# nitishsaDire/objectDetection_ssd

Hardware: AMD Instinct MI355X
Metric: images/sec SSD300-VGG16 train step (higher is better)
Workload: dtype f32 (tensors, accumulators, loss, SGD; the Winograd-domain products of the layers with >= 256 reduction channels are formed from three EXACT bf16 limbs per f32 operand on the bf16 MFMA -- six limb products per f32 product, dropped terms <= 2^-26 -- measured no further from f64 than the f32 MFMA; SSD

## Files before the change

include/ssd_gfx950.h:

```cpp
#ifndef SSD_GFX950_H
#define SSD_GFX950_H

#include <stddef.h>
#include <stdint.h>

#ifdef __cplusplus
extern "C" {
#endif

#define SSD_ABI_VERSION 1

enum ssd_status {
    SSD_OK = 0,
    SSD_ERR_BAD_SHAPE = -1,
    SSD_ERR_WORKSPACE = -2,
    SSD_ERR_NULL = -3,
    SSD_ERR_LAUNCH = -4,
    SSD_ERR_ALIGN = -5
};

int ssd_abi_version(void);
const char* ssd_status_string(int status);

typedef struct ssd_conv_geom {
// ... 24 lines not shown
                          const ssd_conv_geom* g, void* workspace, size_t workspace_bytes, void* stream);
int ssd_tune_set_igemm_bf16(int tile);

int ssd_weight_split_bf16x3(const float* w, void* planes_bf16, size_t n, void* stream);
int ssd_conv2d_fwd_x3(const float* x, const void* w3_ohwi, int w_rows, const float* bias, float* y, int ldy,
                      const ssd_conv_geom* g, int relu, void* stream);
int ssd_conv2d_dgrad_x3(const float* dy, int ldy, const void* w3_ihwo, int Co_pad, float* dx,
                        const float* relu_mask, int accumulate, const ssd_conv_geom* g, void* stream);
int ssd_tune_set_igemm_x3(int tile);
int ssd_conv3x3_halo_fwd_bf16(const float* x, const void* w3_ohwi, int w_rows, const float* bias, float* y, int ldy,
                              const ssd_conv_geom* g, int relu, void* stream);
int ssd_conv3x3_halo_dgrad_bf16(const float* dy, int ldy, const void* w3_ihwo, int Co_pad, float* dx,
                                const float* relu_mask, int accumulate, const ssd_conv_geom* g, void* stream);
int ssd_tune_set_halo(int mode);

int ssd_conv3x3_bf16(const void* x, int ldx, const void* w, int w_rows, int K, const float* bias, void* out, int ldo, int n_out,
                     int out_f32, const void* relu_mask, int accumulate, int relu, int flip, int N, int H, int W, void* stream);
int ssd_tune_set_conv_bf16_mfma(int rows);
int ssd_tune_set_conv_bf16_k64(int on);
int ssd_tune_set_conv_bf16(int mode, int bn);
int ssd_conv3x3_wgrad_bf16t(const void* x_bf16, const void* dy_bf16, int ldy, float* dw_oihw, float* dbias, const ssd_conv_geom* g,
                            void* workspace, size_t workspace_bytes, void* stream);
int ssd_conv1_first_fwd_bf16(const float* x_nchw, const float* w_rows, const float* bias, void* y_nhwc_bf16, int N, int H, int W, int relu,
                             void* stream);
int ssd_conv1_first_wgrad_bf16(const float* x_nchw, const void* dy_nhwc_bf16, float* dw_rows, float* dbias, int N, int H, int W,
                               void* workspace, size_t workspace_bytes, void* stream);
int ssd_maxpool_fwd_bf16(const void* x, void* y, uint8_t* argmax, int N, int H, int W, int C, int k, int stride, int pad, int Ho, int Wo,
                         void* stream);
int ssd_maxpool_bwd_bf16(const void* dy, const uint8_t* argmax, void* dx, const void* relu_mask, const void* y_gate, int accumulate, int N,
                         int H, int W, int C, int k, int stride, int pad, int Ho, int Wo, void* stream);
int ssd_l2norm_fwd_bf16(const void* x, const float* gamma, void* y, int M, int C, void* stream);
size_t ssd_l2norm_bwd_bf16_workspace(int M, int C);
int ssd_l2norm_bwd_bf16(const void* x, const float* gamma, const void* dy, void* dx, float* dgamma, int M, int C, void* workspace,
                        size_t workspace_bytes, void* stream);
int ssd_heads_gather_bf16(const float* dloc, const float* dconf, void* packed_bf16, int ld, int N, int HW, int A, int prior_off, int P,
                          int ncls, void* stream);
int ssd_cast_f32_bf16(const float* x, void* y_bf16, size_t n, void* stream);
int ssd_cast_bf16_f32(const void* x_bf16, float* y, size_t n, void* stream);

size_t ssd_conv2d_wgrad_workspace(const ssd_conv_geom* g);
int ssd_conv2d_wgrad(const float* x, const float* dy, int ldy, float* dw_oihw, float* dbias,
                     const ssd_conv_geom* g, void* workspace, size_t workspace_bytes, void* stream);

int ssd_conv2d_igemm_tile(const ssd_conv_geom* g, int direction, int* bm, int* bn);
int ssd_conv2d_wgrad_tile(const ssd_conv_geom* g, int* bt, int* nsplit);
int ssd_conv2d_wgrad_plan(const ssd_conv_geom* g, int bf16, int* plan);
int ssd_conv3x3_bf16_plan(int N, int H, int W, int K, int n_out, int* plan);
int ssd_conv3x3_halo_shape(const ssd_conv_geom* g, int direction, int planes);
size_t ssd_conv2d_igemm_workspace(const ssd_conv_geom* g, int direction );
int ssd_conv2d_fwd_ws(const float* x, const float* w_ohwi, const float* bias, float* y, int ldy, const ssd_conv_geom* g,
                      int relu, void* workspace, size_t workspace_bytes, void* stream);
int ssd_conv2d_dgrad_ws(const float* dy, int ldy, const float* w_ihwo, int Co_pad, float* dx, const float* relu_mask,
                        int accumulate, const ssd_conv_geom* g, void* workspace, size_t workspace_bytes, void* stream);
int ssd_tune_set_igemm_splitk(int k);
int ssd_wino_weights(const float* w_oihw, float* U_fwd, float* U_bwd, int Co, int Ci, int Co_pad, int mo, void* stream);
size_t ssd_conv3x3_wino_workspace(const ssd_conv_geom* g, int direction , int mo);
int ssd_conv3x3_wino_fwd(const float* x, const float* U_fwd, const float* bias, float* y, int ldy, const ssd_conv_geom* g, int relu,
                         int mo, void* workspace, size_t workspace_bytes, void* stream);
int ssd_conv3x3_wino_dgrad(const float* dy, int ldy, const float* U_bwd, int Co_pad, float* dx, const float* relu_mask,
                           int accumulate, const ssd_conv_geom* g, int mo, void* workspace, size_t workspace_bytes, void* stream);
int ssd_conv3x3_wino_fwd_pool(const float* x, const float* U_fwd, const float* bias, float* y_pooled, uint8_t* argmax,
                              const ssd_conv_geom* g, int ceil_mode, float* planes_keep, void* workspace, size_t workspace_bytes,
                              void* stream);
int ssd_conv3x3_wino_fwd_keep(const float* x, const float* U_fwd, const float* bias, float* y, int ldy, const ssd_conv_geom* g, int relu,
                              float* planes_keep, void* workspace, size_t workspace_bytes, void* stream);
size_t ssd_conv3x3_wino_wgrad_workspace(const ssd_conv_geom* g, int ldy, int mo);
int ssd_conv3x3_wino_wgrad(const float* x, const float* dy, int ldy, float* dw_oihw, float* dbias, const ssd_conv_geom* g, int mo,
                           void* workspace, size_t workspace_bytes, void* stream);
typedef struct ssd_weight_job {
    const float* w0; const float* w1;
    float* out_fwd; float* out_bwd;
    int co0, co, ci, taps, co_pad, kind, pad0, pad1;
} ssd_weight_job;
int ssd_weight_job_blocks(const ssd_weight_job* job);
int ssd_weights_prepare(const ssd_weight_job* jobs_device, const int* block_start_device, int njobs, int total_blocks, void* stream);
size_t ssd_wino4_bias_partial_floats(const ssd_conv_geom* g, int ldy);
int ssd_wino4_dy_transform(const float* dy, int ldy, const ssd_conv_geom* g, float* wgrad_planes, float* dgrad_planes_out,
                           float* bias_partial, void* stream);
size_t ssd_wino4_wgrad_gemm_workspace(const ssd_conv_geom* g, int ldy);
int ssd_wino4_wgrad_gemm(const float* wgrad_planes, const float* x_planes, int ldy, const float* bias_partial, float* dw_oihw, float* dbias,
                         const ssd_conv_geom* g, void* workspace, size_t workspace_bytes, void* stream);
int ssd_wino4_dy_transform_pooled(const float* dpool, const unsigned char* argmax, const float* y_pooled, int Hp, int Wp, int ldy,
                                  const ssd_conv_geom* g, float* wgrad_planes, float* dgrad_planes_out, float* bias_partial, void* stream);
int ssd_conv3x3_wino_wgrad_planes_pooled(const float* planes, const float* dpool, const unsigned char* argmax, const float* y_pooled,
                                         int Hp, int Wp, int ldy, float* dw_oihw, float* dbias, const ssd_conv_geom* g,
                                         float* dgrad_planes_out, void* workspace, size_t workspace_bytes, void* stream);
int ssd_conv3x3_wino_fwd_keep_bits(const float* x, const float* U_fwd, const float* bias, float* y, int ldy, const ssd_conv_geom* g, int relu,
                                   float* planes_keep, uint64_t* relu_bits_out, void* workspace, size_t workspace_bytes, void* stream);
int ssd_conv3x3_wino_fwd_pool_bits(const float* x, const float* U_fwd, const float* bias, float* y_pooled, uint8_t* argmax,
                                   const ssd_conv_geom* g, int ceil_mode, float* planes_keep, uint64_t* relu_bits_out, void* workspace,
                                   size_t workspace_bytes, void* stream);
int ssd_conv3x3_wino_dgrad_bits(const float* dy, int ldy, const float* U_bwd, int Co_pad, float* dx, const uint64_t* relu_bits, int accumulate,
                                const ssd_conv_geom* g, void* workspace, size_t workspace_bytes, void* stream);
int ssd_conv3x3_wino_dgrad_planes_bits(const float* dy_planes, const float* U_bwd, int Co_pad, float* dx, const uint64_t* relu_bits,
                                       int accumulate, const ssd_conv_geom* g, void* workspace, size_t workspace_bytes, void* stream);
int ssd_conv3x3_wino_wgrad_planes(const float* planes, const float* dy, int ldy, float* dw_oihw, float* dbias, const ssd_conv_geom* g,
                                  float* dgrad_planes_out, void* workspace, size_t workspace_bytes, void* stream);
int ssd_conv3x3_wino_dgrad_planes(const float* dy_planes, const float* U_bwd, int Co_pad, float* dx, const float* relu_mask,
                                  int accumulate, const ssd_conv_geom* g, void* workspace, size_t workspace_bytes, void* stream);
int ssd_conv1_first_wino_fwd(const float* x_nchw, const float* w_rows, const float* bias, float* planes, uint64_t* relu_bits, int N, int H, int W,
                             void* stream);
int ssd_conv3x3_wino_fwd_from_planes(const float* planes, const float* U_fwd, const float* bias, float* y, int ldy, float* y_pooled, uint8_t* argmax,
                                     const ssd_conv_geom* g, int relu, int ceil_mode, void* workspace, size_t workspace_bytes, void* stream);
int ssd_wino_weights_adj(const float* w_oihw, float* U_adj, int Co, int Ci, int Co_pad, void* stream);
size_t ssd_wino4_adj_planes_floats(const ssd_conv_geom* g);
int ssd_conv3x3_wino_dgrad_adj_gemm(const float* y_planes, int ldy, const float* U_adj, float* md_planes, const ssd_conv_geom* g, void* stream);
int ssd_wino4_adj_output(const float* md_planes, float* dx, const float* relu_mask, const uint64_t* relu_bits, int accumulate,
                         const ssd_conv_geom* g, void* stream);
int ssd_wino4_adj_output_to_planes(const float* md_planes, const float* relu_mask, const uint64_t* relu_bits, const ssd_conv_geom* g,
                                   const ssd_conv_geom* g_below, float* y_planes, float* bias_partial, void* stream);
int ssd_tune_set_wino_bias_tail(int on);
int ssd_tune_set_wino_xform_blocks(int blocks);
int ssd_tune_set_wino_fused(int mode);
int ssd_gemm_planes_x3v2(const void* a3, const void* w3, float* out, int M, int K, int N, int n_rows, int nbatch, int dither, void* stream);
int ssd_tune_set_x3_big(int mode);
int ssd_tune_set_x3_mfma(int rows);
int ssd_tune_set_gemm_nt(int mode);
int ssd_wino_uses_x3(int mo, int K);
int ssd_tune_set_wino_x3(int on);
size_t ssd_gemm_x3_weights_bytes(int rows, int K, int nbatch);
int ssd_gemm_x3_split_weights(const float* w, void* w3, int rows, int K, int nbatch, void* stream);
int ssd_gemm_planes_x3(const float* a, const void* w3, float* out, int M, int K, int N, int n_rows, int nbatch, void* stream);
int ssd_conv1x1_fwd_x3(const float* x, const void* w3, const float* bias, float* y, int ldy, const ssd_conv_geom* g, int relu, void* stream);
int ssd_conv1x1_dgrad_x3(const float* dy, int ldy, const void* w3t, float* dx, const float* relu_mask, int accumulate, const ssd_conv_geom* g,
                         void* stream);
size_t ssd_conv1x1_wgrad_x3_workspace(const ssd_conv_geom* g, int ldy);
int ssd_conv1x1_wgrad_x3(const float* x, const float* dy, int ldy, float* dw, float* dbias, const ssd_conv_geom* g, void* workspace,
                         size_t workspace_bytes, void* stream);
int ssd_gemm_planes_f32(const float* a, const float* w, float* out, int M, int K, int N, int n_rows, int nbatch, void* stream);
int ssd_has_experimental(void);
int ssd_tune_set_wino_full(int mode);
int ssd_conv3x3_wino_uses_full(const ssd_conv_geom* g, int direction);
int ssd_tune_set_wino_fused_stagger(int cycles);
int ssd_tune_set_wino_fused_stamps(uint64_t* device_buffer);
int ssd_tune_set_wino_wgrad_tn(int on);
int ssd_prof_gemm_begin(void);
int ssd_prof_gemm_collect_kinds(float* ms_out, double* flops_out, int* kinds_out, int max);
int ssd_prof_gemm_collect(float* ms_out, double* flops_out, int max);
int ssd_tune_set_igemm(int tile, int nbuf);
int ssd_tune_set_igemm_stamps(uint64_t* device_buffer);
int ssd_tune_set_dgrad_parity(int on);
int ssd_tune_set_batched_units(int on);
int ssd_tune_set_igemm_lds_pad(int bytes);
int ssd_tune_set_wgrad(int bt, int nbuf, int blocks_per_cu);
int ssd_tune_set_wgrad_patch(int shape);

int ssd_im2col_first(const float* x_nchw, float* out, int N, int H, int W, void* stream);
int ssd_conv1_first_fwd(const float* x_nchw, const float* w_rows, const float* bias, float* y_nhwc, float* col_out, int N, int H, int W,
                        int relu, void* stream);
size_t ssd_conv1_first_wgrad_workspace(int N, int H, int W);
int ssd_conv1_first_wgrad(const float* x_nchw, const float* dy_nhwc, float* dw_rows, float* dbias, int N, int H, int W, void* workspace,
                          size_t workspace_bytes, void* stream);

int ssd_im2col_nchw3(const float* x_nchw, float* out, int N, int H, int W, int R, int S, int stride, int pad,
                     int Ho, int Wo, int Kpad, void* stream);
int ssd_conv2d_fwd_accum(const float* x, const float* w_ohwi, const float* bias, float* y_inout, int ldy,
                         const ssd_conv_geom* g, int relu, void* stream);
int ssd_conv2d_fwd_accum_bf16(const float* x, const float* w_ohwi, const float* bias, float* y_inout, int ldy,
                              const ssd_conv_geom* g, int relu, void* stream);
int ssd_channel_affine(const float* x, const float* scale, const float* shift, float* y, size_t M, int C, int relu,
                       void* stream);

int ssd_maxpool_fwd(const float* x, float* y, uint8_t* argmax, int N, int H, int W, int C,
                    int k, int stride, int pad, int Ho, int Wo, void* stream);
int ssd_maxpool_bwd(const float* dy, const uint8_t* argmax, float* dx, const float* relu_mask, int accumulate,
                    int N, int H, int W, int C, int k, int stride, int pad, int Ho, int Wo, void* stream);
// ... 126 lines not shown
```

objectdetection_ssd_amd/Model.py:

```python
from __future__ import annotations

import numbers
from typing import Dict, List, Optional

import torch
import torch.nn as nn

from . import ops
from .Util import ANCHORS_PER_CELL, ANCHORS_PER_CELL_512, subsampling

N_CLASSES = 21
MAX_FOREGROUND = 255
_VGG_CFG = (64, 64, "M", 128, 128, "M", 256, 256, 256, "M", 512, 512, 512, "M", 512, 512, 512, "M")


class _VGG16(nn.Module):

    def __init__(self):
        super().__init__()
        layers: List[nn.Module] = []
        cin = 3
        for v in _VGG_CFG:
            if v == "M":
                layers.append(nn.MaxPool2d(kernel_size=2, stride=2))
# ... 673 lines not shown
                        return self._timed("dgrad " + pre, "conv3x3_bf16_kernel", ops.conv_flops(g),
                                           lambda: ops.conv3x3_bf16(dy, wb16, None, g.Ci, False, flip=True, out=dx, out_f32=f32_dx, relu_mask=mask,
                                                                    accumulate=acc))
                    deliver(op["x"], dgrad16)
                    continue
                if xin.dtype == torch.bfloat16:
                    xin = T[op["x"] + ":f32"]
                dy = ops.heads_gather(dloc, dconf, co_pad, bs, g.Ho * g.Wo, op["a"], off)
                dyp = None
                dw = db = None
                if any(need[pre + s] for s in ("_bb.weight", "_bb.bias", "_cl.weight", "_cl.bias")):
                    if self._wino_wgrad_ok(g, True) and async_wgrad and side_ctx[0] is None and aux.get("planes:" + pre) is not None \
                            and co_pad <= 1024:
                        kept = aux.pop("planes:" + pre)
                        Y, dyp, part = ops.wino_dy_transform(dy, g, co_pad, True, True)

                        def put(dw, db, pre=pre, a4=a4):
                            grads[pre + "_bb.weight"], grads[pre + "_cl.weight"] = dw[:a4], dw[a4:]
                            grads[pre + "_bb.bias"], grads[pre + "_cl.bias"] = db[:a4], db[a4:]
                        self._wgrad_gemm_async(main, Y, kept, part, g, co_pad, put)
                        wgrad_used = True
                    elif self._wino_wgrad_ok(g, True):
                        kept = aux.pop("planes:" + pre, None)
                        dual = kept is not None and self.dual_dy
                        res = self._timed("wgrad " + pre, "winograd_3x3", ops.wino_flops(g),
                                          lambda: ops.conv2d_wgrad_wino(xin, dy, g, co_pad, True, mo=self.WINO_TILE, planes=kept,
                                                                        dgrad_planes=dual, dw_out=self._gout(pre + "_bb.weight", pre + "_cl.weight"),
                                                                        db_out=self._gout(pre + "_bb.bias", pre + "_cl.bias")))
                        dw, db = res[0], res[1]
                        dyp = res[2] if dual else None
                    else:
                        def wg(pre=pre, a4=a4, xin=xin, dy=dy, g=g, co_pad=co_pad):
                            dw_, db_ = self._timed("wgrad " + pre, ops.wgrad_tile(g, self.bf16) if self.prof is not None else "", ops.conv_flops(g),
                                                   lambda: ops.conv2d_wgrad(xin, dy, g, co_pad, True, bf16=self.bf16,
                                                                            dw_out=self._gout(pre + "_bb.weight", pre + "_cl.weight"),
                                                                            db_out=self._gout(pre + "_bb.bias", pre + "_cl.bias")))
                            grads[pre + "_bb.weight"], grads[pre + "_cl.weight"] = dw_[:a4], dw_[a4:]
                            grads[pre + "_bb.bias"], grads[pre + "_cl.bias"] = db_[:a4], db_[a4:]
                        if side_ctx[0] is not None and defer:
                            deferred.append(wg)
                        else:
                            wg()
                    if dw is not None:
                        grads[pre + "_bb.weight"], grads[pre + "_cl.weight"] = dw[:a4], dw[a4:]
                        grads[pre + "_bb.bias"], grads[pre + "_cl.bias"] = db[:a4], db[a4:]
                if self._wino_ok(g):
                    _, ub = self._wino_weights(pre, (P[pre + "_bb.weight"], P[pre + "_cl.weight"]), co_pad)
                    deliver(op["x"], lambda dx, acc, mask: self._timed("dgrad " + pre, "winograd_3x3", ops.wino_flops(g),
                                                                       lambda: ops.conv2d_dgrad_wino(dy, ub, g, dx, mask, acc, planes=dyp)))
                    continue
                _, wb = self._layouts(pre, (P[pre + "_bb.weight"], P[pre + "_cl.weight"]), co_pad, True)
                deliver(op["x"], lambda dx, acc, mask: self._timed(
                    "dgrad " + pre, ops.igemm_tile(g, 1, self.bf16, self.x3) if self.prof is not None else "", ops.conv_flops(g),
                    lambda: ops.conv2d_dgrad_x3(dy, wb, g, dx, mask, acc) if self.x3 else
                    ops.conv2d_dgrad(dy, wb, g, dx, mask, acc, bf16=self.bf16, w3=self._planes(pre, True))))
            elif kind == "conv":
                dy = G.pop(op["y"])
                g = aux[op["y"]]
                xin = T[op["x"]]
                dyp = None
                if self._t16(g, xin) and dy.dtype == torch.bfloat16:
                    name = op["p"]
                    if need[name + ".weight"] or need[name + ".bias"]:
                        grads[name + ".weight"], grads[name + ".bias"] = self._timed(
                            "wgrad " + name, "wgrad3x3_bf16_kernel", ops.conv_flops(g),
                            lambda: ops.conv3x3_wgrad_bf16t(xin, dy, g, g.Co, True, dw_out=self._gout(name + ".weight"), db_out=self._gout(name + ".bias")))
                    _, wb16 = self._bf16_weights(name, (P[name + ".weight"],))
                    deliver(op["x"], lambda dx, acc, mask: self._timed(
                        "dgrad " + name, "conv3x3_bf16_kernel", ops.conv_flops(g),
                        lambda: ops.conv3x3_bf16(dy, wb16, None, g.Ci, False, flip=True, out=dx, relu_mask=mask, accumulate=acc)))
                    continue
                to_bf16 = xin.dtype == torch.bfloat16
                if to_bf16:
                    xin = T[op["x"] + ":f32"]
                if isinstance(dy, ops.PooledGrad):
                    if not ((need[op["p"] + ".weight"] or need[op["p"] + ".bias"]) and self._wino_wgrad_ok(g, False) and self.WINO_TILE == 4
                            and self.dual_dy and aux.get("planes:" + op["p"]) is not None and g.Co % 32 == 0 and g.Co <= 1024
                            and not ops.wino_uses_full(g, 1) and self._wino_ok(g)):
                        dy = dy.materialize()
                adj = (self._adj_ok(g) and not to_bf16 and aux.get("planes:" + op["p"]) is not None and not (async_wgrad and side_ctx[0] is None)
                       and not ops.wino_uses_full(g, 1))
                if isinstance(dy, ops.AdjPlanesGrad) and not adj:
                    dy = dy.materialize()
                if adj:
                    name = op["p"]
                    kept = aux.pop("planes:" + name)
                    need_w = need[name + ".weight"] or need[name + ".bias"]

                    def dy_planes(dy=dy, g=g, need_w=need_w):
                        if isinstance(dy, ops.AdjPlanesGrad):
                            return ops.wino_adj_output_to_planes(dy.md, dy.g, g, dy.relu_mask, dy.bits, want_bias=need_w)
                        Yp, _, part = ops.wino_dy_transform(dy, g, g.Co, False, need_w)
                        return Yp, part
                    if need_w:
                        def wg_adj(name=name, g=g, kept=kept):
                            Yp, part = dy_planes()
                            dw_, db_ = ops.wino_wgrad_gemm(Yp, kept, part, g, g.Co, dw_out=self._gout(name + ".weight"), db_out=self._gout(name + ".bias"))
                            return Yp, dw_, db_
                        Y, dw, db = self._timed("wgrad " + name, "winograd_3x3", ops.wino_flops(g), wg_adj)
                        grads[name + ".weight"], grads[name + ".bias"] = dw, db
                    else:
                        Y, _ = dy_planes()
                    del kept
                    _, uadj = self._wino_weights(name, (P[name + ".weight"],), op["co"], adj=True)
                    bits = aux.pop("bits:" + name, None)
                    below = self._conv_of.get(op["x"]) if self.adjoint_chain else None
                    gb = aux.get(op["x"]) if below is not None else None
                    chain = (below is not None and gb is not None and self.consumers[op["x"]] == 1 and op["x"] in self.relu_out
                             and self._adj_ok(gb) and aux.get("planes:" + below["p"]) is not None and gb.Co == g.Ci
                             and (gb.N, gb.H, gb.W) == (g.N, g.H, g.W) and T[op["x"]].dtype == torch.float32)

                    def dgrad_adj(dx, acc, mask, Y=Y, uadj=uadj, g=g, bits=bits, chain=chain):
                        md = ops.wino_dgrad_adj_gemm(Y, uadj, g, g.Co)
                        use_bits = bits if mask is not None else None
                        fmask = None if use_bits is not None else mask
                        if chain and dx is None and not acc and mask is not None:
                            return ops.AdjPlanesGrad(md, g, fmask, use_bits)
                        return ops.wino_adj_output(md, g, dx, relu_mask=fmask, bits=use_bits, accumulate=acc)
                    deliver(op["x"], lambda dx, acc, mask: self._timed("dgrad " + name, "winograd_3x3", ops.wino_flops(g),
                                                                       lambda: dgrad_adj(dx, acc, mask)))
                    continue
                if need[op["p"] + ".weight"] or need[op["p"] + ".bias"]:
                    if self._wino_wgrad_ok(g, False) and async_wgrad and side_ctx[0] is None and aux.get("planes:" + op["p"]) is not None \
                            and g.Co % 32 == 0 and g.Co <= 1024:
                        kept = aux.pop("planes:" + op["p"])
                        Y, dyp, part = ops.wino_dy_transform(dy, g, g.Co, not ops.wino_uses_full(g, 1), True)

                        def put(dw, db, name=op["p"]):
                            grads[name + ".weight"], grads[name + ".bias"] = dw, db
                        self._wgrad_gemm_async(main, Y, kept, part, g, g.Co, put)
                        wgrad_used = True
                        dw = None
                    elif self._wino_wgrad_ok(g, False):
                        kept = aux.pop("planes:" + op["p"], None)
                        dual = kept is not None and self.dual_dy and g.Co % 32 == 0 and not ops.wino_uses_full(g, 1)
                        res = self._timed("wgrad " + op["p"], "winograd_3x3", ops.wino_flops(g),
                                          lambda: ops.conv2d_wgrad_wino(xin, dy, g, g.Co, True, mo=self.WINO_TILE, planes=kept,
                                                                        dgrad_planes=dual, dw_out=self._gout(op["p"] + ".weight"),
                                                                        db_out=self._gout(op["p"] + ".bias")))
                        dw, db = res[0], res[1]
                        dyp = res[2] if dual else None
                    else:
                        def wg(name=op["p"], xin=xin, dy=dy, g=g):
                            if self._x31_ok(g):
                                grads[name + ".weight"], grads[name + ".bias"] = self._timed(
                                    "wgrad " + name, "gemm_tn_x3_kernel (1x1)", ops.conv_flops(g),
                                    lambda: ops.conv1x1_wgrad_x3(xin, dy, g, g.Co, True, dw_out=self._gout(name + ".weight"),
                                                                 db_out=self._gout(name + ".bias")))
                                return
                            grads[name + ".weight"], grads[name + ".bias"] = self._timed(
                                "wgrad " + name, ops.wgrad_tile(g, self.bf16) if self.prof is not None else "", ops.conv_flops(g),
                                lambda: ops.conv2d_wgrad(xin, dy, g, g.Co, True, bf16=self.bf16, dw_out=self._gout(name + ".weight"),
                                                         db_out=self._gout(name + ".bias")))
                        if side_ctx[0] is not None and defer:
                            deferred.append(wg)
                        else:
                            wg()
                        dw = None
                    if dw is not None:
                        grads[op["p"] + ".weight"], grads[op["p"] + ".bias"] = dw, db
                if self._wino_ok(g):
                    _, ub = self._wino_weights(op["p"], (P[op["p"] + ".weight"],), op["co"], adj=self._adj_ok(g))
                    if self._adj_ok(g):
                        raise RuntimeError(f"{op['p']}: its filter planes are laid out for the adjoint data gradient, which needs the forward's kept planes "
                                           "(the engine's keep_planes / dual_dy / adjoint_dgrad switches must not change between a forward and its backward)")
                    bits = aux.pop("bits:" + op["p"], None) if (dyp is not None or ops.wino_uses_full(g, 1) or isinstance(T[op["x"]], _Elided)) else None
                    def dgrad_rot(dx, acc, mask, dy=dy, ub=ub, g=g, dyp=dyp, bits=bits, name=op["p"]):
                        if isinstance(mask, _Elided):
                            if bits is None:
                                raise RuntimeError(f"{name}: its input was not stored and no ReLU bits were kept for its data gradient")
                            mask_t = None
                        else:
                            mask_t = mask
                        return ops.conv2d_dgrad_wino(None if isinstance(dy, ops.PooledGrad) else dy, ub, g, dx, mask_t, acc, planes=dyp,
                                                     bits=bits if mask is not None else None)
                    deliver(op["x"], lambda dx, acc, mask: self._timed("dgrad " + op["p"], "winograd_3x3", ops.wino_flops(g),
                                                                       lambda: dgrad_rot(dx, acc, mask)))
                    continue
                if self._x31_ok(g) and not to_bf16:
                    _, w3b = self._x31_weights(op["p"], (P[op["p"] + ".weight"],), op["co"])
                    deliver(op["x"], lambda dx, acc, mask: self._timed(
                        "dgrad " + op["p"], "gemm_planes_x3_kernel (1x1)", ops.conv_flops(g),
                        lambda: ops.conv1x1_dgrad_x3(dy, w3b, g, dx, mask, acc)))
                    continue
                _, wb = self._layouts(op["p"], (P[op["p"] + ".weight"],), op["co"], True)
                if to_bf16:
                    def boundary(dx, acc, mask, dy=dy, wb=wb, g=g, name=op["p"]):
                        if acc or mask is not None or dx is not None:
                            raise RuntimeError("the bf16 trunk's boundary tensor must have one consumer and no ReLU of its own")
                        d32 = self._timed("dgrad " + name, ops.igemm_tile(g, 1, self.bf16, self.x3) if self.prof is not None else "", ops.conv_flops(g),
                                          lambda: ops.conv2d_dgrad(dy, wb, g, None, None, False, bf16=self.bf16, w3=self._planes(name, True)))
                        return ops.cast_bf16(d32)
                    deliver(op["x"], boundary)
                    continue
                deliver(op["x"], lambda dx, acc, mask: self._timed(
                    "dgrad " + op["p"], ops.igemm_tile(g, 1, self.bf16, self.x3) if self.prof is not None else "", ops.conv_flops(g),
                    lambda: ops.conv2d_dgrad_x3(dy, wb, g, dx, mask, acc) if self.x3 else
                    ops.conv2d_dgrad(dy, wb, g, dx, mask, acc, bf16=self.bf16, w3=self._planes(op["p"], True))))
            elif kind == "pool":
                dy = G.pop(op["y"])
                xin = T[op["x"]]
                am = aux[op["y"]]
                yout = T[op["y"]]
                deliver(op["x"], lambda dx, acc, mask: (
                    ops.PooledGrad(dy, am, yout, xin.shape)
                    if (self.lazy_pool_grad and isinstance(xin, _Elided) and mask is not None and not acc and dx is None
                        and (op["k"], op["s"], op["pad"]) == (2, 2, 0)) else
                    ops.maxpool_bwd(dy, am, tuple(xin.shape), op["k"], op["s"], op["pad"], dx, y_gate=yout)
                    if (mask is not None and not acc) else
                    ops.maxpool_bwd(dy, am, tuple(xin.shape), op["k"], op["s"], op["pad"], dx, mask, acc)))
            elif kind == "l2norm":
                dy = G.pop(op["y"])
                xin = T[op["x"]]
                gamma = P[op["p"]].detach().reshape(-1)
                box = {}

                def run(dx, acc, mask, xin=xin, gamma=gamma, dy=dy, box=box):
                    if acc or mask is not None:
                        raise RuntimeError("L2-norm backward must deliver the first, non-final gradient of its input")
                    dx, box["dg"] = ops.l2norm_bwd(xin, gamma, dy, dg_out=self._gout(op["p"]))
                    return dx
                deliver(op["x"], run)
                grads[op["p"]] = box["dg"].reshape(P[op["p"]].shape)
            elif kind == "conv_first":
                dy = G.pop(op["y"])
                if need[op["p"] + ".weight"] or need[op["p"] + ".bias"]:
                    g = aux[op["y"]]
                    col = T["x_col"]
                    if col is None:
                        dw, db = self._timed("wgrad " + op["p"], "conv_first_wgrad_kernel", 2.0 * dy.numel() * 27,
                                             lambda: (ops.conv1_first_wgrad_bf16 if dy.dtype == torch.bfloat16 else ops.conv1_first_wgrad)(T["x"], dy, True))
                    else:
                        dw, db = self._timed("wgrad " + op["p"], ops.wgrad_tile(g, self.bf16) if self.prof is not None else "", 2.0 * dy.numel() * 27,
                                             lambda: ops.conv2d_wgrad(col, dy, g, g.Co, True))
                    grads[op["p"] + ".weight"], grads[op["p"] + ".bias"] = ops.first_weight_grad(dw), db
        if not joined:
            main.wait_event(join_event)
        if side_done is not None:
            main.wait_event(side_done)
        if wgrad_used:
            main.wait_event(self._wgrad_stream.record_event())
        if held:
            grads.release()
        return grads


class _SSD300Function(torch.autograd.Function):
    @staticmethod
    def forward(ctx, x, engine, *params):
        P = dict(zip(engine.names, params))
        loc, conf, saved = engine.forward(x, P, save=True)
        ctx.engine = engine
        ctx.saved = saved
        ctx.params = params
        return loc, conf

    @staticmethod
    def backward(ctx, dloc, dconf):
        eng = ctx.engine
        P = dict(zip(eng.names, ctx.params))
        need = {n: bool(f) for n, f in zip(eng.names, ctx.needs_input_grad[2:])}
        grads = eng.backward(ctx.saved, dloc, dconf, P, need)
        ctx.saved = None
        if eng.sink_owns_grads and eng.grad_sink is not None:
            return (None, None) + (None,) * len(eng.names)
        return (None, None) + tuple(grads.get(n) if need[n] else None for n in eng.names)


def _check_n_classes(n_classes) -> int:
    if isinstance(n_classes, bool) or not isinstance(n_classes, numbers.Integral):
        raise ValueError(f"n_classes must be an integer, got {n_classes!r}")
    if not 1 <= int(n_classes) <= MAX_FOREGROUND:
        raise ValueError(f"n_classes must be in 1..{MAX_FOREGROUND} (foreground classes; background is added), got {n_classes}")
    return int(n_classes)


class SSD_300(nn.Module):
    _VARIANT = 300

    def __init__(self, *, n_classes: int = 20):
        super().__init__()
        self.n_classes = _check_n_classes(n_classes)
        n_conf = self.n_classes + 1
        self.model = _VGG16()
        self.rescaling_conv_4_3 = nn.Parameter(torch.full((1, 512, 1, 1), 20.))
        feats = self.model.features
        self.conv_4_3 = nn.Sequential(*feats[0:16], nn.MaxPool2d(2, 2, 0, 1, ceil_mode=True), *feats[17:23])
        self.seq5 = nn.Sequential(*feats[23:30], nn.MaxPool2d(3, 1, 1, 1, ceil_mode=True))
        cls0, cls3 = self.model.classifier[0], self.model.classifier[3]
        self.fc6 = subsampling(cls0.weight.detach().view(4096, 512, 7, 7), [4, None, 3, 3])
# ... 129 lines not shown
```

objectdetection_ssd_amd/_lib.py:

```python
from __future__ import annotations

import ctypes as C
import os

PKG = os.path.dirname(os.path.abspath(__file__))
LIB_PATH = os.path.join(PKG, "libssd_gfx950.so")

SSD_ABI_VERSION = 1


class ConvGeom(C.Structure):
    _fields_ = [(n, C.c_int32) for n in ("N", "H", "W", "Ci", "Ho", "Wo", "Co", "R", "S", "stride", "pad", "dil")]


class ImageDesc(C.Structure):
    _fields_ = [("src_offset", C.c_int64)] + [(n, C.c_int32) for n in (
        "src_h", "src_w", "canvas_h", "canvas_w", "place_top", "place_left", "crop_top", "crop_left", "crop_h", "crop_w",
        "flip", "reserved")]


class WeightJob(C.Structure):
    _fields_ = [("w0", C.c_void_p), ("w1", C.c_void_p), ("out_fwd", C.c_void_p), ("out_bwd", C.c_void_p)] + [(n, C.c_int32) for n in (
        "co0", "co", "ci", "taps", "co_pad", "kind", "pad0", "pad1")]

# ... 28 lines not shown
    "ssd_tune_set_igemm_x3": (_I, [_I]),
    "ssd_tune_set_halo": (_I, [_I]),
    "ssd_clock_probe": (_I, [_P, _P]),
    "ssd_tune_set_x3_mfma": (_I, [_I]),
    "ssd_tune_set_x3_big": (_I, [_I]),
    "ssd_tune_set_loss_form": (_I, [_I]),
    "ssd_gemm_planes_x3v2": (_I, [_P, _P, _P, _I, _I, _I, _I, _I, _I, _P]),
    "ssd_graph_node_counts": (_I, [_P, _P, _P]),
    "ssd_photometric_workspace": (_Z, [_I]),
    "ssd_photometric_u8": (_I, [_P, _P, _P, _P, _P, _I, _P, _Z, _P]),
    "ssd_preprocess_workspace": (_Z, [_P, _I, _I, _I]),
    "ssd_preprocess_u8": (_I, [_P, _P, _P, _I, _I, _I, _P, _P, _P, _P, _P, _Z, _P]),
    "ssd_map_eval_workspace": (_Z, [_I, _I]),
    "ssd_map_eval": (_I, [_P, _P, _P, _P, _I, _P, _P, _P, _I, _I, _I, _P, _I, _P, _P, _P, _P, _Z, _P]),
    "ssd_eval_match_workspace": (_Z, [_I]),
    "ssd_eval_match": (_I, [_P, _P, _P, _P, _P, _I, _I, _P, _P, _P, _P, _I, _I, _I, _P, _I, _P, _P, _P, _P, _P, _Z, _P]),
    "ssd_eval_ap_workspace": (_Z, [_I]),
    "ssd_eval_ap": (_I, [_P, _P, _P, _P, _I, _P, _I, _I, _I, _P, _P, _P, _Z, _P]),
    "ssd_coco_match_workspace": (_Z, [_I]),
    "ssd_coco_match": (_I, [_P, _P, _P, _P, _P, _I, _I, _P, _P, _P, _P, _P, _I, _I, _I, _P, _I, _P, _P, _I, _I, _P, _P, _P, _P, _P, _P,
                            _Z, _P]),
    "ssd_coco_ap_workspace": (_Z, [_I]),
    "ssd_coco_ap": (_I, [_P, _P, _P, _P, _P, _I, _P, _I, _I, _I, _P, _I, _P, _P, _P, _P, _Z, _P]),
    "ssd_im2col_nchw3": (_I, [_P, _P, _I, _I, _I, _I, _I, _I, _I, _I, _I, _I, _P]),
    "ssd_conv2d_fwd_accum": (_I, [_P, _P, _P, _P, _I, _G, _I, _P]),
    "ssd_conv2d_fwd_accum_bf16": (_I, [_P, _P, _P, _P, _I, _G, _I, _P]),
    "ssd_channel_affine": (_I, [_P, _P, _P, _P, C.c_size_t, _I, _I, _P]),
    "ssd_conv3x3_bf16": (_I, [_P, _I, _P, _I, _I, _P, _P, _I, _I, _I, _P, _I, _I, _I, _I, _I, _I, _P]),
    "ssd_tune_set_conv_bf16": (_I, [_I, _I]),
    "ssd_tune_set_conv_bf16_k64": (_I, [_I]),
    "ssd_tune_set_conv_bf16_mfma": (_I, [_I]),
    "ssd_wino_uses_x3": (_I, [_I, _I]),
    "ssd_tune_set_wino_x3": (_I, [_I]),
    "ssd_gemm_x3_weights_bytes": (_Z, [_I, _I, _I]),
    "ssd_gemm_x3_split_weights": (_I, [_P, _P, _I, _I, _I, _P]),
    "ssd_gemm_planes_x3": (_I, [_P, _P, _P, _I, _I, _I, _I, _I, _P]),
    "ssd_gemm_planes_f32": (_I, [_P, _P, _P, _I, _I, _I, _I, _I, _P]),
    "ssd_conv1x1_fwd_x3": (_I, [_P, _P, _P, _P, _I, _G, _I, _P]),
    "ssd_conv1x1_dgrad_x3": (_I, [_P, _I, _P, _P, _P, _I, _G, _P]),
    "ssd_conv1x1_wgrad_x3_workspace": (_Z, [_G, _I]),
    "ssd_conv1x1_wgrad_x3": (_I, [_P, _P, _I, _P, _P, _G, _P, _Z, _P]),
    "ssd_has_experimental": (_I, []),
    "ssd_conv3x3_wgrad_bf16t": (_I, [_P, _P, _I, _P, _P, _G, _P, _Z, _P]),
    "ssd_conv1_first_fwd_bf16": (_I, [_P, _P, _P, _P, _I, _I, _I, _I, _P]),
    "ssd_conv1_first_wgrad_bf16": (_I, [_P, _P, _P, _P, _I, _I, _I, _P, _Z, _P]),
    "ssd_maxpool_fwd_bf16": (_I, [_P, _P, _P, _I, _I, _I, _I, _I, _I, _I, _I, _I, _P]),
    "ssd_maxpool_bwd_bf16": (_I, [_P, _P, _P, _P, _P, _I, _I, _I, _I, _I, _I, _I, _I, _I, _I, _P]),
    "ssd_l2norm_fwd_bf16": (_I, [_P, _P, _P, _I, _I, _P]),
    "ssd_l2norm_bwd_bf16_workspace": (_Z, [_I, _I]),
    "ssd_l2norm_bwd_bf16": (_I, [_P, _P, _P, _P, _P, _I, _I, _P, _Z, _P]),
    "ssd_heads_gather_bf16": (_I, [_P, _P, _P, _I, _I, _I, _I, _I, _I, _I, _P]),
    "ssd_cast_f32_bf16": (_I, [_P, _P, _Z, _P]),
    "ssd_cast_bf16_f32": (_I, [_P, _P, _Z, _P]),
    "ssd_conv3x3_halo_fwd_bf16": (_I, [_P, _P, _I, _P, _P, _I, _G, _I, _P]),
    "ssd_conv3x3_halo_dgrad_bf16": (_I, [_P, _I, _P, _I, _P, _P, _I, _G, _P]),
    "ssd_conv2d_wgrad_workspace": (_Z, [_G]),
    "ssd_conv2d_wgrad": (_I, [_P, _P, _I, _P, _P, _G, _P, _Z, _P]),
    "ssd_conv2d_igemm_tile": (_I, [_G, _I, C.POINTER(C.c_int), C.POINTER(C.c_int)]),
    "ssd_conv2d_wgrad_tile": (_I, [_G, C.POINTER(C.c_int), C.POINTER(C.c_int)]),
    "ssd_conv2d_wgrad_plan": (_I, [_G, _I, C.POINTER(C.c_int)]),
    "ssd_conv3x3_bf16_plan": (_I, [_I, _I, _I, _I, _I, C.POINTER(C.c_int)]),
    "ssd_conv3x3_halo_shape": (_I, [_G, _I, _I]),
    "ssd_conv2d_igemm_workspace": (_Z, [_G, _I]),
    "ssd_conv2d_fwd_ws": (_I, [_P, _P, _P, _P, _I, _G, _I, _P, _Z, _P]),
    "ssd_conv2d_dgrad_ws": (_I, [_P, _I, _P, _I, _P, _P, _I, _G, _P, _Z, _P]),
    "ssd_tune_set_igemm_splitk": (_I, [_I]),
    "ssd_wino_weights": (_I, [_P, _P, _P, _I, _I, _I, _I, _P]),
    "ssd_conv3x3_wino_workspace": (_Z, [_G, _I, _I]),
    "ssd_conv3x3_wino_fwd": (_I, [_P, _P, _P, _P, _I, _G, _I, _I, _P, _Z, _P]),
    "ssd_conv3x3_wino_fwd_pool": (_I, [_P, _P, _P, _P, _P, _G, _I, _P, _P, _Z, _P]),
    "ssd_conv3x3_wino_fwd_keep": (_I, [_P, _P, _P, _P, _I, _G, _I, _P, _P, _Z, _P]),
    "ssd_weight_job_blocks": (_I, [_P]),
    "ssd_weights_prepare": (_I, [_P, _P, _I, _I, _P]),
    "ssd_wino4_bias_partial_floats": (_Z, [_G, _I]),
    "ssd_wino4_dy_transform": (_I, [_P, _I, _G, _P, _P, _P, _P]),
    "ssd_wino_weights_adj": (_I, [_P, _P, _I, _I, _I, _P]),
    "ssd_conv1_first_wino_fwd": (_I, [_P, _P, _P, _P, _P, _I, _I, _I, _P]),
    "ssd_conv3x3_wino_fwd_from_planes": (_I, [_P, _P, _P, _P, _I, _P, _P, _G, _I, _I, _P, _Z, _P]),
    "ssd_wino4_adj_planes_floats": (_Z, [_G]),
    "ssd_conv3x3_wino_dgrad_adj_gemm": (_I, [_P, _I, _P, _P, _G, _P]),
    "ssd_wino4_adj_output": (_I, [_P, _P, _P, _P, _I, _G, _P]),
    "ssd_wino4_adj_output_to_planes": (_I, [_P, _P, _P, _G, _G, _P, _P, _P]),
    "ssd_wino4_dy_transform_pooled": (_I, [_P, _P, _P, _I, _I, _I, _G, _P, _P, _P, _P]),
    "ssd_conv3x3_wino_wgrad_planes_pooled": (_I, [_P, _P, _P, _P, _I, _I, _I, _P, _P, _G, _P, _P, _Z, _P]),
    "ssd_wino4_wgrad_gemm_workspace": (_Z, [_G, _I]),
    "ssd_wino4_wgrad_gemm": (_I, [_P, _P, _I, _P, _P, _P, _G, _P, _Z, _P]),
    "ssd_conv3x3_wino_fwd_keep_bits": (_I, [_P, _P, _P, _P, _I, _G, _I, _P, _P, _P, _Z, _P]),
    "ssd_conv3x3_wino_fwd_pool_bits": (_I, [_P, _P, _P, _P, _P, _G, _I, _P, _P, _P, _Z, _P]),
    "ssd_conv3x3_wino_dgrad_planes_bits": (_I, [_P, _P, _I, _P, _P, _I, _G, _P, _Z, _P]),
    "ssd_conv3x3_wino_wgrad_planes": (_I, [_P, _P, _I, _P, _P, _G, _P, _P, _Z, _P]),
    "ssd_conv3x3_wino_dgrad_planes": (_I, [_P, _P, _I, _P, _P, _I, _G, _P, _Z, _P]),
    "ssd_conv3x3_wino_dgrad": (_I, [_P, _I, _P, _I, _P, _P, _I, _G, _I, _P, _Z, _P]),
    "ssd_conv3x3_wino_wgrad_workspace": (_Z, [_G, _I, _I]),
    "ssd_conv3x3_wino_wgrad": (_I, [_P, _P, _I, _P, _P, _G, _I, _P, _Z, _P]),
    "ssd_tune_set_wino_wgrad_tn": (_I, [_I]),
    "ssd_tune_set_wino_fused": (_I, [_I]),
    "ssd_tune_set_gemm_nt": (_I, [_I]),
    "ssd_tune_set_wino_bias_tail": (_I, [_I]),
    "ssd_tune_set_batched_units": (_I, [_I]),
    "ssd_tune_set_dgrad_parity": (_I, [_I]),
    "ssd_tune_set_wino_full": (_I, [_I]),
    "ssd_conv3x3_wino_uses_full": (_I, [_G, _I]),
    "ssd_conv3x3_wino_dgrad_bits": (_I, [_P, _I, _P, _I, _P, _P, _I, _G, _P, _Z, _P]),
    "ssd_tune_set_wino_xform_blocks": (_I, [_I]),
    "ssd_tune_set_wino_fused_stamps": (_I, [_P]),
    "ssd_tune_set_wino_fused_stagger": (_I, [_I]),
    "ssd_prof_gemm_begin": (_I, []),
    "ssd_prof_gemm_collect": (_I, [_P, _P, _I]),
    "ssd_prof_gemm_collect_kinds": (_I, [_P, _P, _P, _I]),
    "ssd_tune_set_igemm": (_I, [_I, _I]),
    "ssd_tune_set_igemm_lds_pad": (_I, [_I]),
    "ssd_tune_set_igemm_stamps": (_I, [_P]),
    "ssd_tune_set_wgrad": (_I, [_I, _I, _I]),
    "ssd_tune_set_wgrad_patch": (_I, [_I]),
    "ssd_im2col_first": (_I, [_P, _P, _I, _I, _I, _P]),
    "ssd_conv1_first_fwd": (_I, [_P, _P, _P, _P, _P, _I, _I, _I, _I, _P]),
    "ssd_conv1_first_wgrad_workspace": (_Z, [_I, _I, _I]),
    "ssd_conv1_first_wgrad": (_I, [_P, _P, _P, _P, _I, _I, _I, _P, _Z, _P]),
    "ssd_maxpool_fwd": (_I, [_P, _P, _P, _I, _I, _I, _I, _I, _I, _I, _I, _I, _P]),
    "ssd_maxpool_bwd_gated": (_I, [_P, _P, _P, _P, _I, _I, _I, _I, _I, _I, _I, _I, _I, _P]),
    "ssd_maxpool_bwd": (_I, [_P, _P, _P, _P, _I, _I, _I, _I, _I, _I, _I, _I, _I, _I, _P]),
    "ssd_l2norm_fwd": (_I, [_P, _P, _P, _I, _I, _P]),
    "ssd_l2norm_bwd_workspace": (_Z, [_I, _I]),
    "ssd_l2norm_bwd": (_I, [_P, _P, _P, _P, _P, _I, _I, _P, _Z, _P]),
    "ssd_heads_scatter": (_I, [_P, _I, _P, _P, _I, _I, _I, _I, _I, _I, _P]),
    "ssd_heads_gather": (_I, [_P, _P, _P, _I, _I, _I, _I, _I, _I, _I, _P]),
    "ssd_multibox_loss_workspace": (_Z, [_I, _I, _I]),
    "ssd_multibox_loss": (_I, [_P, _P, _P, _P, _P, _I, _I, _P, _P, _I, _I, _F, _I, _I, _P, _P, _P, _P, _P, _P, _Z, _P]),
    "ssd_decode_nms_workspace": (_Z, [_I, _I]),
    "ssd_decode_nms": (_I, [_P, _P, _P, _I, _I, _F, _F, _I, _F, _F, _P, _P, _P, _P, _P, _P, _Z, _P]),
    "ssd_decode_nms_batch_workspace": (_Z, [_I, _I, _I]),
    "ssd_decode_nms_batch": (_I, [_P, _P, _P, _P, _I, _I, _I, _F, _F, _I, _P, _P, _P, _P, _P, _P, _Z, _P]),
    "ssd_decode_nms_soft": (_I, [_P, _P, _P, _I, _I, _F, _F, _I, _F, _F, _P, _P, _P, _P, _P, _P, _Z, _P, _I, _F, _F]),
    "ssd_decode_nms_batch_soft": (_I, [_P, _P, _P, _P, _I, _I, _I, _F, _F, _I, _P, _P, _P, _P, _P, _P, _Z, _P, _I, _F, _F]),
    "ssd_soft_nms_sorted": (_I, [_P, _P, _P, _I, _I, _I, _I, _F, _F, _F, _I, _P, _P, _P, _P]),
    "ssd_sgd_momentum": (_I, [_P, _P, _P, _Z, _F, _F, _F, _P, _I, _P]),
    "ssd_bn_workspace": (_Z, [_Z, _I]),
    "ssd_bn_train_stats": (_I, [_P, _I, _Z, _I, _P, _P, _F, _F, _P, _P, _P, _P, _P, _P, _P, _P, _Z, _P]),
    "ssd_bn_apply": (_I, [_P, _I, _Z, _I, _P, _P, _P, _I, _P, _P, _I, _I, _F, _U64, _I, _I, _P, _I, _P]),
    "ssd_bn_train_bwd": (_I, [_P, _I, _P, _I, _Z, _I, _P, _P, _P, _I, _F, _U64, _I, _I, _I, _P, _P, _P, _I, _P, _I, _P, _Z, _P]),
    "ssd_dropout_mask": (_I, [_P, _Z, _F, _U64, _I, _P]),
}

_lib = None


def load() -> C.CDLL:
    global _lib
    if _lib is not None:
        return _lib
    import torch
    if not os.path.exists(LIB_PATH):
        from . import build as _build
        _build.build()
    try:
        lib = C.CDLL(LIB_PATH)
    except OSError as e:
        raise RuntimeError(f"cannot load {LIB_PATH}: {e}.  The gfx950 HIP extension is the only compute "
                           f"path of this package; build it with `python -m objectdetection_ssd_amd.build`.") from e
    for name, (res, args) in SIGNATURES.items():
        fn = getattr(lib, name)
        fn.restype = res
        fn.argtypes = args
    if lib.ssd_abi_version() != SSD_ABI_VERSION:
        raise RuntimeError("libssd_gfx950.so ABI version mismatch; rebuild")
    _lib = lib
# ... 8 lines not shown
```

objectdetection_ssd_amd/csrc/gemm_x3.hip:

```cpp
#include <type_traits>
#include "common.h"

int ssd_internal_prof_open(double flops, int kind, hipStream_t st);
void ssd_internal_prof_close(int slot, hipStream_t st);

namespace {

typedef __bf16 bf16x8 __attribute__((ext_vector_type(8)));
typedef unsigned int u32x4 __attribute__((ext_vector_type(4)));
typedef __attribute__((address_space(3))) void lds_void;

constexpr unsigned OOB = 0xFFFFFF00u;

struct GemmX3Params {
    const float* __restrict__ a;
    const __bf16* __restrict__ w3;
    float* __restrict__ out;
    int M, K, N, rows_pad;
    int tiles_m, tiles_n, nbatch;
    size_t batch_a, batch_out;
    const float* __restrict__ bias;
    const float* __restrict__ mask;
    int ldo, relu, accumulate;
};
// ... 714 lines not shown
    p.batch_a = batch_a_elems; p.batch_out = (size_t)M * N;
    const size_t nblk = (size_t)p.tiles_m * p.tiles_n * nbatch;
    if (nblk >= (1ull << 31)) return SSD_ERR_BAD_SHAPE;
    if (K >= 64 && N % 4 == 0 && ((g_x3_big == 1 && N >= 256 && M >= 2048) || g_x3_big == 2)) {
        const size_t nblk2 = (size_t)ssd_cdiv(M, 256) * ssd_cdiv(N, 256) * nbatch;
        const int slot2 = ssd_internal_prof_open(6.0 * 2.0 * (double)nblk2 * 256.0 * 256.0 * K, 4, st);
        const int e = ssd_internal_gemm_batched_x3s(a, w3, out, M, K, N, n_rows, nbatch, batch_a_elems, st);
        ssd_internal_prof_close(slot2, st);
        return e;
    }
    const int slot = ssd_internal_prof_open(6.0 * 2.0 * (double)nblk * 128.0 * 128.0 * K, 4, st);
#ifdef X3_PIPE
    {
        static std::atomic<unsigned long long> raised{0};
        int dev;
        if (ssd_attr_needed(raised, dev)) {
            (void)hipFuncSetAttribute(reinterpret_cast<const void*>(gemm_planes_x3p_kernel<false>), hipFuncAttributeMaxDynamicSharedMemorySize, 0);
            ssd_attr_done(raised, dev);
        }
    }
    hipLaunchKernelGGL(gemm_planes_x3p_kernel<false>, dim3((unsigned)nblk), dim3(256), 0, st, p);
#else
#ifdef SSD_EXPERIMENTAL
    if (g_x3_m16) hipLaunchKernelGGL((gemm_planes_x3_kernel<false, true>), dim3((unsigned)nblk), dim3(256), 0, st, p);
    else
#endif
    hipLaunchKernelGGL((gemm_planes_x3_kernel<false, false>), dim3((unsigned)nblk), dim3(256), 0, st, p);
#endif
    ssd_internal_prof_close(slot, st);
    SSD_CHECK_LAUNCH();
    return SSD_OK;
}

extern "C" int ssd_tune_set_x3_big(int mode) {
    if (mode < 0 || mode > 2) return SSD_ERR_BAD_SHAPE;
#ifndef SSD_EXPERIMENTAL
    if (mode != 0) return SSD_ERR_BAD_SHAPE;
#endif
    g_x3_big = mode;
    return SSD_OK;
}

extern "C" int ssd_tune_set_x3_mfma(int rows) {
    if (rows != 16 && rows != 32) return SSD_ERR_BAD_SHAPE;
#ifndef SSD_EXPERIMENTAL
    if (rows == 16) return SSD_ERR_BAD_SHAPE;
#endif
    g_x3_m16 = rows == 16;
    return SSD_OK;
}

__attribute__((visibility("hidden"))) int ssd_internal_gemm_tn_x3(const float* a, const float* c, float* out, int M, int N, int K, int lda, int ldc,
                                                                   int nbatch, int ksplit, int ksteps_per_split, size_t batch_a, size_t batch_c,
                                                                   hipStream_t st) {
    if (M <= 0 || N <= 0 || K <= 0 || lda % 4 != 0 || ldc % 4 != 0 || nbatch <= 0 || ksplit < 1 || ksteps_per_split < 1) return SSD_ERR_BAD_SHAPE;
    if ((size_t)ksplit * ksteps_per_split * 16 < (size_t)K) return SSD_ERR_BAD_SHAPE;
    if (batch_a * 4 >= 0xF0000000ull || batch_c * 4 >= 0xF0000000ull) return SSD_ERR_BAD_SHAPE;
    TnX3Params q{};
    q.a = a; q.c = c; q.out = out;
    q.M = M; q.N = N; q.K = K; q.lda = lda; q.ldc = ldc;
    q.tiles_m = ssd_cdiv(M, 128); q.tiles_n = ssd_cdiv(N, 128);
    q.ksplit = ksplit; q.ksteps_per_split = ksteps_per_split; q.groups = nbatch * ksplit;
    q.batch_a = batch_a; q.batch_c = batch_c;
    q.a_bytes = (unsigned)((size_t)K * lda * 4); q.c_bytes = (unsigned)((size_t)K * ldc * 4);
    const size_t nblk = (size_t)q.tiles_m * q.tiles_n * q.groups;
    if (nblk >= (1ull << 31)) return SSD_ERR_BAD_SHAPE;
    const int slot = ssd_internal_prof_open(6.0 * 2.0 * (double)nblk * 128.0 * 128.0 * 16.0 * ksteps_per_split, 5, st);
    hipLaunchKernelGGL(gemm_tn_x3_kernel, dim3((unsigned)nblk), dim3(256), 0, st, q);
    ssd_internal_prof_close(slot, st);
    SSD_CHECK_LAUNCH();
    return SSD_OK;
}

namespace {
__global__ __launch_bounds__(256) void x3_slab_sum_kernel(const float* __restrict__ slab, float* __restrict__ out, size_t n4, int nslab) {
    for (size_t i = (size_t)blockIdx.x * 256 + threadIdx.x; i < n4; i += (size_t)gridDim.x * 256) {
        f32x4 sum = *reinterpret_cast<const f32x4*>(slab + i * 4);
        for (int k = 1; k < nslab; ++k) sum += *reinterpret_cast<const f32x4*>(slab + (size_t)k * n4 * 4 + i * 4);
        *reinterpret_cast<f32x4*>(out + i * 4) = sum;
    }
}
__global__ __launch_bounds__(256) void x3_colsum_partial_kernel(const float* __restrict__ dy, float* __restrict__ part, size_t M, int ld) {
    const int q4 = ld >> 2;
    for (int q = threadIdx.x; q < q4; q += 256) {
        f32x4 s0 = {0.f, 0.f, 0.f, 0.f};
        for (size_t m = blockIdx.x; m < M; m += gridDim.x) s0 += *reinterpret_cast<const f32x4*>(dy + m * ld + q * 4);
        *reinterpret_cast<f32x4*>(part + (size_t)blockIdx.x * ld + q * 4) = s0;
    }
}
__global__ __launch_bounds__(256) void x3_colsum_final_kernel(const float* __restrict__ part, float* __restrict__ db, int nblk, int C, int ld) {
    __shared__ float red[4][64];
    const int cl = threadIdx.x & 63, q = threadIdx.x >> 6;
    const int c = blockIdx.x * 64 + cl;
    float t = 0.f;
    if (c < C)
        for (int k = q; k < nblk; k += 4) t += part[(size_t)k * ld + c];
    red[q][cl] = t;
    __syncthreads();
    if (q == 0 && c < C) db[c] = ((red[0][cl] + red[1][cl]) + red[2][cl]) + red[3][cl];
}
constexpr int X3_COLSUM_BLOCKS = 256;
struct X3WgradPlan { int ks, per; size_t slab_floats, part_floats; };
X3WgradPlan x3_wgrad_plan(const ssd_conv_geom* g, int ldy) {
    X3WgradPlan w;
    const size_t M = (size_t)g->N * g->Ho * g->Wo;
    const int tiles = ssd_cdiv(g->Co, 128) * ssd_cdiv(g->Ci, 128), steps16 = (int)((M + 15) / 16);
    int ks = 768 / tiles;
    if (ks > 1) ks &= ~1;
    if (ks > steps16 / 8) ks = steps16 / 8;
    if (ks < 1) ks = 1;
    w.per = ssd_cdiv(steps16, ks);
    w.ks = ssd_cdiv(steps16, w.per);
    w.slab_floats = (size_t)w.ks * g->Co * g->Ci;
    w.part_floats = (size_t)X3_COLSUM_BLOCKS * ldy;
    return w;
}
bool x3_1x1_geom_ok(const ssd_conv_geom* g) {
    return g && g->R == 1 && g->S == 1 && g->stride == 1 && g->pad == 0 && g->Ho == g->H && g->Wo == g->W && g->N > 0 && g->H > 0 && g->W > 0 &&
           g->Ci > 0 && g->Co > 0;
}
}

extern "C" int ssd_conv1x1_fwd_x3(const float* x, const void* w3, const float* bias, float* y, int ldy, const ssd_conv_geom* g, int relu, void* stream) {
    if (!x || !w3 || !y) return SSD_ERR_NULL;
    if (!x3_1x1_geom_ok(g) || g->Ci % 32 != 0 || ldy < g->Co) return SSD_ERR_BAD_SHAPE;
    if (!ssd_aligned16(x) || !ssd_aligned16(w3) || !ssd_aligned16(y)) return SSD_ERR_ALIGN;
    const size_t M = (size_t)g->N * g->H * g->W;
    if (M >= (1ull << 31) || M * g->Ci * 4 >= 0xF0000000ull) return SSD_ERR_BAD_SHAPE;
    GemmX3Params p{};
    p.a = x; p.w3 = static_cast<const __bf16*>(w3); p.out = y;
    p.M = (int)M; p.K = g->Ci; p.N = g->Co; p.rows_pad = ssd_cdiv(g->Co, 128) * 128;
    p.tiles_m = ssd_cdiv((int)M, 128); p.tiles_n = ssd_cdiv(g->Co, 128); p.nbatch = 1;
    p.bias = bias; p.mask = nullptr; p.ldo = ldy; p.relu = relu; p.accumulate = 0;
    hipLaunchKernelGGL(gemm_planes_x3_kernel<true>, dim3((unsigned)(p.tiles_m * p.tiles_n)), dim3(256), 0, (hipStream_t)stream, p);
    SSD_CHECK_LAUNCH();
    return SSD_OK;
}

extern "C" int ssd_conv1x1_dgrad_x3(const float* dy, int ldy, const void* w3t, float* dx, const float* relu_mask, int accumulate,
                                    const ssd_conv_geom* g, void* stream) {
    if (!dy || !w3t || !dx) return SSD_ERR_NULL;
    if (!x3_1x1_geom_ok(g) || ldy % 32 != 0 || ldy < g->Co) return SSD_ERR_BAD_SHAPE;
    if (!ssd_aligned16(dy) || !ssd_aligned16(w3t) || !ssd_aligned16(dx) || (relu_mask && !ssd_aligned16(relu_mask))) return SSD_ERR_ALIGN;
    const size_t M = (size_t)g->N * g->H * g->W;
    if (M >= (1ull << 31) || M * ldy * 4 >= 0xF0000000ull) return SSD_ERR_BAD_SHAPE;
    GemmX3Params p{};
    p.a = dy; p.w3 = static_cast<const __bf16*>(w3t); p.out = dx;
    p.M = (int)M; p.K = ldy; p.N = g->Ci; p.rows_pad = ssd_cdiv(g->Ci, 128) * 128;
    p.tiles_m = ssd_cdiv((int)M, 128); p.tiles_n = ssd_cdiv(g->Ci, 128); p.nbatch = 1;
    p.bias = nullptr; p.mask = relu_mask; p.ldo = g->Ci; p.relu = 0; p.accumulate = accumulate;
    hipLaunchKernelGGL(gemm_planes_x3_kernel<true>, dim3((unsigned)(p.tiles_m * p.tiles_n)), dim3(256), 0, (hipStream_t)stream, p);
    SSD_CHECK_LAUNCH();
    return SSD_OK;
}

extern "C" size_t ssd_conv1x1_wgrad_x3_workspace(const ssd_conv_geom* g, int ldy) {
    if (!x3_1x1_geom_ok(g) || ldy < g->Co || ldy % 4 != 0) return 0;
    const X3WgradPlan w = x3_wgrad_plan(g, ldy);
    return (w.slab_floats + w.part_floats) * 4 + 256;
}

extern "C" int ssd_conv1x1_wgrad_x3(const float* x, const float* dy, int ldy, float* dw, float* dbias, const ssd_conv_geom* g, void* workspace,
                                    size_t workspace_bytes, void* stream) {
    if (!x || !dy || !dw || !workspace) return SSD_ERR_NULL;
    if (!x3_1x1_geom_ok(g) || g->Ci % 4 != 0 || ldy % 4 != 0 || ldy < g->Co) return SSD_ERR_BAD_SHAPE;
    if (!ssd_aligned16(x) || !ssd_aligned16(dy) || !ssd_aligned16(dw) || !ssd_aligned16(workspace)) return SSD_ERR_ALIGN;
    if (workspace_bytes < ssd_conv1x1_wgrad_x3_workspace(g, ldy)) return SSD_ERR_WORKSPACE;
    hipStream_t st = (hipStream_t)stream;
    const X3WgradPlan w = x3_wgrad_plan(g, ldy);
    const size_t M = (size_t)g->N * g->H * g->W;
    if (M >= (1ull << 31)) return SSD_ERR_BAD_SHAPE;
    float* slab = static_cast<float*>(workspace);
    float* part = slab + w.slab_floats;
    float* dst = w.ks == 1 && (g->Co * (size_t)g->Ci) % 4 == 0 ? dw : slab;
    if (int e = ssd_internal_gemm_tn_x3(dy, x, dst, g->Co, g->Ci, (int)M, ldy, g->Ci, 1, w.ks, w.per, M * ldy, M * g->Ci, st)) return e;
    if (dst != dw) {
        const size_t n = (size_t)g->Co * g->Ci;
        if (n % 4 != 0) return SSD_ERR_BAD_SHAPE;
        const size_t blocks = (n / 4 + 255) / 256;
// ... 17 lines not shown
```

objectdetection_ssd_amd/csrc/winograd.hip:

```cpp
#include <cstdlib>
#include "common.h"

int ssd_internal_gemm_batched(const float* a, const float* w, float* out, int M, int K, int N, int n_rows, int nbatch,
                              size_t batch_a_elems, size_t batch_w_elems, int ksplit, hipStream_t st);
int ssd_internal_gemm_batched_x3(const float* a, const void* w3, float* out, int M, int K, int N, int n_rows, int nbatch, size_t batch_a_elems,
                                 hipStream_t st);
int ssd_internal_gemm_tn_x3(const float* a, const float* c, float* out, int M, int N, int K, int lda, int ldc, int nbatch, int ksplit,
                            int ksteps_per_split, size_t batch_a, size_t batch_c, hipStream_t st);
int ssd_internal_wino4_gemm_out(const float* V, const float* U, int tiles, int K, int Nrows, int Nout, float* out, int ldo, int Cvalid,
                                const float* bias, const float* mask, const unsigned long long* mask_bits, int relu, int accumulate, int H,
                                int W, int TH, int TW, float* yp, uint8_t* am, int Ho, int Wo, hipStream_t st);

int ssd_internal_wino4_full(const float* x, const float* U, int tiles, int K, int Nrows, int Nout, float* out, int ldo, int Cvalid,
                            const float* bias, const float* mask, const unsigned long long* mask_bits, int relu, int accumulate, int H, int W,
                            int TH, int TW, float* yp, uint8_t* am, int Ho, int Wo, float* V_keep, unsigned long long* bits_out, hipStream_t st);

namespace {

struct Lat { int D; int h0[4], w0[4]; };
__device__ __forceinline__ void lat_tile(const int (&first)[4], int D, int t, int& off, int& base) {
    off = 0;
#pragma unroll
    for (int a = 1; a < 4; ++a)
        if (a < D && t >= first[a]) off = a;
    base = 4 * (t - first[off]);
}

__global__ void wino_weight_kernel(const float* __restrict__ w, float* __restrict__ U, int Co, int Ci, int Nrows, int K, int mode) {
    const size_t total = (size_t)Nrows * K;
    for (size_t i = (size_t)blockIdx.x * blockDim.x + threadIdx.x; i < total; i += (size_t)gridDim.x * blockDim.x) {
        const int k = (int)(i % K), n = (int)(i / K);
        const int co = mode == 0 ? n : k, ci = mode == 0 ? k : n;
        float g[3][3];
#pragma unroll
        for (int r = 0; r < 3; ++r)
#pragma unroll
            for (int s = 0; s < 3; ++s)
                g[r][s] = (co < Co && ci < Ci) ? w[((size_t)co * Ci + ci) * 9 + (mode != 1 ? r * 3 + s : (2 - r) * 3 + (2 - s))] : 0.f;
        float t[4][3];
#pragma unroll
        for (int s = 0; s < 3; ++s) {
            t[0][s] = g[0][s];
            t[1][s] = 0.5f * (g[0][s] + g[1][s] + g[2][s]);
            t[2][s] = 0.5f * (g[0][s] - g[1][s] + g[2][s]);
            t[3][s] = g[2][s];
        }
#pragma unroll
        for (int r = 0; r < 4; ++r) {
            const float u0 = t[r][0], u1 = 0.5f * (t[r][0] + t[r][1] + t[r][2]), u2 = 0.5f * (t[r][0] - t[r][1] + t[r][2]), u3 = t[r][2];
            U[((size_t)(r * 4 + 0) * Nrows + n) * K + k] = u0;
            U[((size_t)(r * 4 + 1) * Nrows + n) * K + k] = u1;
            U[((size_t)(r * 4 + 2) * Nrows + n) * K + k] = u2;
            U[((size_t)(r * 4 + 3) * Nrows + n) * K + k] = u3;
        }
    }
}

__global__ __launch_bounds__(256) void wino_input_kernel(const float* __restrict__ x, float* __restrict__ V, int N, int H, int W, int C,
                                                         int TH, int TW) {
    const int C4 = C >> 2;
    const size_t tiles = (size_t)N * TH * TW, total = tiles * C4;
    for (size_t i = (size_t)blockIdx.x * 256 + threadIdx.x; i < total; i += (size_t)gridDim.x * 256) {
        const int c4 = (int)(i % C4);
        const size_t tile = i / C4;
        const int tw = (int)(tile % TW), th = (int)((tile / TW) % TH), n = (int)(tile / ((size_t)TW * TH));
        f32x4 d[4][4];
#pragma unroll
        for (int a = 0; a < 4; ++a) {
            const int ih = 2 * th - 1 + a;
#pragma unroll
            for (int b = 0; b < 4; ++b) {
                const int iw = 2 * tw - 1 + b;
                const bool ok = (unsigned)ih < (unsigned)H && (unsigned)iw < (unsigned)W;
                d[a][b] = ok ? *reinterpret_cast<const f32x4*>(x + (((size_t)n * H + ih) * W + iw) * C + c4 * 4) : f32x4{0.f, 0.f, 0.f, 0.f};
            }
        }
        f32x4 t[4][4];
#pragma unroll
        for (int b = 0; b < 4; ++b) {
            t[0][b] = d[0][b] - d[2][b];
            t[1][b] = d[1][b] + d[2][b];
            t[2][b] = d[2][b] - d[1][b];
            t[3][b] = d[1][b] - d[3][b];
// ... 464 lines not shown
                        const f32x4 v = y[r][2 * pb + q];
#pragma unroll
                        for (int e = 0; e < 4; ++e)
                            if (first || v[e] > best[e] || v[e] != v[e]) {
                                best[e] = v[e];
                                bi[e] = r * 2 + q;
                            }
                        first = false;
                    }
                }
                const size_t o = (((size_t)n * Ho + oh) * Wo + ow) * C4 + c4;
                *reinterpret_cast<f32x4*>(yp + o * 4) = best;
                if (am != nullptr)
                    *reinterpret_cast<uint32_t*>(am + o * 4) =
                        (uint32_t)bi[0] | ((uint32_t)bi[1] << 8) | ((uint32_t)bi[2] << 16) | ((uint32_t)bi[3] << 24);
            }
        }
    }
}

template <int MODE>
__global__ __launch_bounds__(256) void wino4_xform_t_kernel(const float* __restrict__ src, float* __restrict__ dst, int N, int H, int W, int C,
                                                            int TH, int TW, int Tpad) {
    __shared__ float tr[6][32][33];
    const int C4 = C >> 2;
    const int cgroups = (C4 + 7) / 8;
    const size_t tiles = (size_t)N * TH * TW;
    const int tile_blocks = Tpad / 32;
    const int q = threadIdx.x & 7, tl = threadIdx.x >> 3;
    for (int blk = blockIdx.x; blk < tile_blocks * cgroups; blk += gridDim.x) {
        const int cg = blk % cgroups;
        const size_t tile0 = (size_t)(blk / cgroups) * 32, tile = tile0 + tl;
        const int c4 = cg * 8 + q;
        const bool live = tile < tiles && c4 < C4;
        const int tw = live ? (int)(tile % TW) : 0, th = live ? (int)((tile / TW) % TH) : 0, n = live ? (int)(tile / ((size_t)TW * TH)) : 0;
        f32x4 t[6][6];
        constexpr int NS = MODE == 0 ? 6 : 4;
#pragma unroll
        for (int b2 = 0; b2 < NS; ++b2) {
            f32x4 d[NS];
#pragma unroll
            for (int a = 0; a < NS; ++a) {
                const int ih = MODE == 0 ? 4 * th - 1 + a : 4 * th + a, iw = MODE == 0 ? 4 * tw - 1 + b2 : 4 * tw + b2;
                const bool ok = live && (unsigned)ih < (unsigned)H && (unsigned)iw < (unsigned)W;
                d[a] = ok ? *reinterpret_cast<const f32x4*>(src + (((size_t)n * H + ih) * W + iw) * C + c4 * 4) : f32x4{0.f, 0.f, 0.f, 0.f};
            }
#pragma unroll
            for (int a = 0; a < 6; ++a) {
                f32x4 acc = {0.f, 0.f, 0.f, 0.f};
#pragma unroll
                for (int k = 0; k < NS; ++k) {
                    const float cf = MODE == 0 ? W4_BT[a][k] : W4_AT[k][a];
                    if (cf != 0.f) acc += cf * d[k];
                }
                t[a][b2] = acc;
            }
        }
#pragma unroll
        for (int a = 0; a < 6; ++a) {
            __syncthreads();
#pragma unroll
            for (int b2 = 0; b2 < 6; ++b2) {
                f32x4 acc = {0.f, 0.f, 0.f, 0.f};
#pragma unroll
                for (int k = 0; k < NS; ++k) {
                    const float cf = MODE == 0 ? W4_BT[b2][k] : W4_AT[k][b2];
                    if (cf != 0.f) acc += cf * t[a][k];
                }
#pragma unroll
                for (int e = 0; e < 4; ++e) tr[b2][q * 4 + e][tl] = acc[e];
            }
            __syncthreads();
#pragma unroll
            for (int it = 0; it < 24; ++it) {
                const int row = it * 8 + (threadIdx.x >> 5), col = threadIdx.x & 31;
                const int b2 = row >> 5, cl = row & 31;
                const int c = cg * 32 + cl;
                if (c < C) dst[((size_t)(a * 6 + b2) * C + c) * Tpad + tile0 + col] = tr[b2][cl][col];
            }
        }
    }
}

struct PoolSrc { const uint8_t* am; const float* gate; int Hp, Wp; };
template <bool BIAS, bool POOLED = false>
__global__ __launch_bounds__(256) void wino4_dy_kernel(const float* __restrict__ dy, float* __restrict__ Y, int N, int H, int W, int C,
                                                       int TH, int TW, float* __restrict__ part, int Cvalid, float* __restrict__ Vd,
                                                       const PoolSrc ps, const Lat lat) {
    const int C4 = C >> 2;
    f32x4 bsum = {0.f, 0.f, 0.f, 0.f};
    const size_t tiles = (size_t)N * TH * TW, total = tiles * C4;
    const size_t plane = tiles * C;
    for (size_t i = (size_t)blockIdx.x * 256 + threadIdx.x; i < total; i += (size_t)gridDim.x * 256) {
        const int c4 = (int)(i % C4);
        const size_t tile = i / C4;
        const int tw = (int)(tile % TW), th = (int)((tile / TW) % TH), n = (int)(tile / ((size_t)TW * TH));
        int offh, bh, offw, bw;
        lat_tile(lat.h0, lat.D, th, offh, bh);
        lat_tile(lat.w0, lat.D, tw, offw, bw);
        f32x4 pg[4][4];
        uint32_t pc[4][4];
        if (POOLED) {
#pragma unroll
            for (int r = 0; r < 4; ++r)
#pragma unroll
                for (int q = 0; q < 4; ++q) {
                    const bool inner = (r == 1 || r == 2) && (q == 1 || q == 2);
                    const int ph = 2 * th - 1 + r, pw = 2 * tw - 1 + q;
                    const bool ok = (inner || Vd != nullptr) && (unsigned)ph < (unsigned)ps.Hp && (unsigned)pw < (unsigned)ps.Wp;
                    f32x4 d = {0.f, 0.f, 0.f, 0.f};
                    uint32_t a = 0xffffffffu;
                    if (ok) {
                        const size_t idx = (((size_t)n * ps.Hp + ph) * ps.Wp + pw) * C4 + c4;
                        d = *reinterpret_cast<const f32x4*>(dy + idx * 4);
                        const f32x4 yv = *reinterpret_cast<const f32x4*>(ps.gate + idx * 4);
                        a = *reinterpret_cast<const uint32_t*>(ps.am + idx * 4);
#pragma unroll
                        for (int e = 0; e < 4; ++e) d[e] = yv[e] > 0.f ? d[e] : 0.f;
                    }
                    pg[r][q] = d;
                    pc[r][q] = a;
                }
        }
        auto patch = [&](int a, int b) -> f32x4 {
            const int lh = bh - 1 + a, lw = bw - 1 + b;
            const int ih = lat.D * lh + offh, iw = lat.D * lw + offw;
            const bool ok = lh >= 0 && lw >= 0 && ih < H && iw < W;
            if (!POOLED)
                return ok ? *reinterpret_cast<const f32x4*>(dy + (((size_t)n * H + ih) * W + iw) * C + c4 * 4) : f32x4{0.f, 0.f, 0.f, 0.f};
            const int r = (a + 1) >> 1, q = (b + 1) >> 1;
            const uint32_t code = (uint32_t)(((a + 1) & 1) * 2 + ((b + 1) & 1));
            f32x4 g;
#pragma unroll
            for (int e = 0; e < 4; ++e) g[e] = (ok && ((pc[r][q] >> (8 * e)) & 0xffu) == code) ? pg[r][q][e] : 0.f;
            return g;
        };
        if (Vd != nullptr) {
            f32x4 u[6][6];
#pragma unroll
            for (int b = 0; b < 6; ++b) {
                f32x4 d[6];
#pragma unroll
                for (int a = 0; a < 6; ++a) d[a] = patch(a, b);
#pragma unroll
                for (int a = 0; a < 6; ++a) {
                    f32x4 acc = {0.f, 0.f, 0.f, 0.f};
#pragma unroll
                    for (int k = 0; k < 6; ++k)
                        if (W4_BT[a][k] != 0.f) acc += W4_BT[a][k] * d[k];
                    u[a][b] = acc;
                }
            }
            float* dv = Vd + tile * C + c4 * 4;
#pragma unroll
            for (int a = 0; a < 6; ++a)
#pragma unroll
                for (int b = 0; b < 6; ++b) {
                    f32x4 acc = {0.f, 0.f, 0.f, 0.f};
#pragma unroll
                    for (int k = 0; k < 6; ++k)
                        if (W4_BT[b][k] != 0.f) acc += W4_BT[b][k] * u[a][k];
                    *reinterpret_cast<f32x4*>(dv + (size_t)(a * 6 + b) * plane) = acc;
                }
        }
        f32x4 t[6][4];
#pragma unroll
        for (int b = 0; b < 4; ++b) {
            f32x4 d[4];
#pragma unroll
            for (int a = 0; a < 4; ++a) d[a] = patch(a + 1, b + 1);
            if (BIAS) bsum += (d[0] + d[1]) + (d[2] + d[3]);
#pragma unroll
            for (int a = 0; a < 6; ++a) {
                f32x4 acc = {0.f, 0.f, 0.f, 0.f};
#pragma unroll
                for (int k = 0; k < 4; ++k)
                    if (W4_AT[k][a] != 0.f) acc += W4_AT[k][a] * d[k];
                t[a][b] = acc;
            }
        }
        float* dst = Y + tile * C + c4 * 4;
#pragma unroll
        for (int a = 0; a < 6; ++a)
#pragma unroll
            for (int b = 0; b < 6; ++b) {
                f32x4 acc = {0.f, 0.f, 0.f, 0.f};
#pragma unroll
                for (int k = 0; k < 4; ++k)
                    if (W4_AT[k][b] != 0.f) acc += W4_AT[k][b] * t[a][k];
                *reinterpret_cast<f32x4*>(dst + (size_t)(a * 6 + b) * plane) = acc;
            }
    }
    if (BIAS) {
        __shared__ f32x4 red[256];
        red[threadIdx.x] = bsum;
        __syncthreads();
        if ((int)threadIdx.x < C4) {
            f32x4 t = red[threadIdx.x];
            for (int k = threadIdx.x + C4; k < 256; k += C4) t += red[k];
            const int c4 = (int)(((size_t)blockIdx.x * 256 + threadIdx.x) % C4);
#pragma unroll
            for (int e = 0; e < 4; ++e)
                if (c4 * 4 + e < Cvalid) part[(size_t)blockIdx.x * ((Cvalid + 3) / 4 * 4) + c4 * 4 + e] = t[e];
        }
    }
}

template <bool MAKE_Y, bool BIAS>
__global__ __launch_bounds__(256) void wino4_adj_out_kernel(const float* __restrict__ Md, int N, int H, int W, int C, int TH, int TW,
                                                            float* __restrict__ dx, int ldo, const float* __restrict__ mask,
                                                            const unsigned long long* __restrict__ mask_bits, int accumulate,
                                                            float* __restrict__ Y, float* __restrict__ part, int Cvalid) {
    const int C4 = C >> 2;
    f32x4 bsum = {0.f, 0.f, 0.f, 0.f};
    const size_t tiles = (size_t)N * TH * TW, total = tiles * C4;
// ... 151 lines not shown
                if (c4 * 4 + e < Cvalid) part[(size_t)blockIdx.x * ((Cvalid + 3) / 4 * 4) + c4 * 4 + e] = t[e];
        }
    }
}

struct TnParams {
    const float* a; const float* b; float* out;
    int M, N, K, lda, ldb, tiles_m, tiles_n, ksplit, ksteps_per_split, groups;
    size_t batch_a, batch_b;
    unsigned a_bytes, b_bytes;
};
constexpr int TN_LD = 96;
__device__ __forceinline__ f32x4 tn_load16(__amdgpu_buffer_rsrc_t srd, unsigned voff) {
    return __builtin_bit_cast(f32x4, __builtin_amdgcn_raw_buffer_load_b128(srd, (int)voff, 0, 0));
}
__global__ __launch_bounds__(256) void wino_gemm_tn_kernel(const TnParams p) {
    __shared__ __attribute__((aligned(16))) float lds[2 * 32 * TN_LD];
    float* As = lds;
    float* Bs = lds + 32 * TN_LD;
    const int tid = threadIdx.x, lane = tid & 63, wave = tid >> 6;
    const int wm = wave >> 1, wn = wave & 1;
    const int nblk = p.tiles_m * p.tiles_n;
    const int idx = (int)(blockIdx.x >> 3), grp = (idx / nblk) * 8 + (int)(blockIdx.x & 7), lid = idx % nblk;
    if (grp >= p.groups) return;
    const int m0 = (lid / p.tiles_n) * 64, n0 = (lid % p.tiles_n) * 64;
    const int by = grp % p.ksplit, bz = grp / p.ksplit;
    const __amdgpu_buffer_rsrc_t srd_a = __builtin_amdgcn_make_buffer_rsrc(const_cast<float*>(p.a + (size_t)bz * p.batch_a), 0, (int)p.a_bytes, 0x00020000);
    const __amdgpu_buffer_rsrc_t srd_b = __builtin_amdgcn_make_buffer_rsrc(const_cast<float*>(p.b + (size_t)bz * p.batch_b), 0, (int)p.b_bytes, 0x00020000);
    const int mchunk = tid & 15, krow = tid >> 4;
    const unsigned OOB = 0xFFFFFFF0u;
    const int col_a = m0 + mchunk * 4, col_b = n0 + mchunk * 4;
    const bool ok_a = col_a < p.lda, ok_b = col_b < p.ldb;
    const int ksteps = (p.K + 31) / 32;
    const int kt_begin = by * p.ksteps_per_split;
    const int KT = min(ksteps - kt_begin, p.ksteps_per_split);

    f32x16 acc;
#pragma unroll
    for (int r = 0; r < 16; ++r) acc[r] = 0.f;
    f32x4 ra[2], rb[2];
    auto issue = [&](int kt) {
        const int k0 = (kt_begin + kt) * 32 + krow;
#pragma unroll
        for (int j = 0; j < 2; ++j) {
            ra[j] = tn_load16(srd_a, ok_a ? (unsigned)(((size_t)(k0 + 16 * j) * p.lda + col_a) * 4) : OOB);
            rb[j] = tn_load16(srd_b, ok_b ? (unsigned)(((size_t)(k0 + 16 * j) * p.ldb + col_b) * 4) : OOB);
        }
    };
    auto store = [&]() {
#pragma unroll
        for (int j = 0; j < 2; ++j) {
            *reinterpret_cast<f32x4*>(&As[(krow + 16 * j) * TN_LD + mchunk * 4]) = ra[j];
            *reinterpret_cast<f32x4*>(&Bs[(krow + 16 * j) * TN_LD + mchunk * 4]) = rb[j];
        }
    };
    const int lr = lane & 31, lh = lane >> 5;
    const int a_rd = lh * TN_LD + wm * 32 + lr, b_rd = lh * TN_LD + wn * 32 + lr;
    if (KT > 0) {
        issue(0);
        store();
    }
    __syncthreads();
    for (int kt = 0; kt < KT; ++kt) {
        const bool more = kt + 1 < KT;
        if (more) issue(kt + 1);
#pragma unroll
        for (int q = 0; q < 16; ++q)
            acc = __builtin_amdgcn_mfma_f32_32x32x2f32(As[a_rd + 2 * q * TN_LD], Bs[b_rd + 2 * q * TN_LD], acc, 0, 0, 0);
        __syncthreads();
        if (more) {
            store();
            __syncthreads();
        }
    }
    float* out = p.out + ((size_t)bz * p.ksplit + by) * p.M * p.N;
    const int n = n0 + wn * 32 + lr;
#pragma unroll
    for (int r = 0; r < 16; ++r) {
        const int m = m0 + wm * 32 + (r & 3) + 8 * (r >> 2) + 4 * lh;
        if (m < p.M && n < p.N) out[(size_t)m * p.N + n] = acc[r];
    }
}

__global__ __launch_bounds__(256) void wino_splitk_sum_kernel(float* __restrict__ Zs, size_t total, int P, int ksplit) {
    const size_t quads = total >> 2, n = quads * P;
    for (size_t idx = (size_t)blockIdx.x * 256 + threadIdx.x; idx < n; idx += (size_t)gridDim.x * 256) {
        const size_t pl = idx / quads, q = idx - pl * quads;
        float* src = Zs + pl * ksplit * total + q * 4;
        f32x4 sum = *reinterpret_cast<const f32x4*>(src);
        for (int k = 1; k < ksplit; ++k) sum += *reinterpret_cast<const f32x4*>(src + (size_t)k * total);
        *reinterpret_cast<f32x4*>(src) = sum;
    }
}

__global__ __launch_bounds__(256) void wino4_wgrad_finish_kernel(const float* __restrict__ Zs, float* __restrict__ dw, int Co, int Ci, int ksplit,
                                                                 size_t pstride, int nfin, const BiasTail bt) {
    if ((int)blockIdx.x >= nfin) {
        colsum_final4_body(bt.part, bt.db, bt.nblk, bt.C, bt.ldp, (int)blockIdx.x - nfin);
        return;
    }
    const size_t total = (size_t)Co * Ci, quads = total >> 2;
    for (size_t q = (size_t)blockIdx.x * 256 + threadIdx.x; q < quads; q += (size_t)nfin * 256) {
        const size_t i = q * 4;
        f32x4 z[6][6];
#pragma unroll
        for (int pl = 0; pl < 36; ++pl) z[pl / 6][pl % 6] = *reinterpret_cast<const f32x4*>(Zs + (size_t)pl * pstride + i);
        for (int k = 1; k < ksplit; ++k)
#pragma unroll
            for (int pl = 0; pl < 36; ++pl) z[pl / 6][pl % 6] += *reinterpret_cast<const f32x4*>(Zs + (size_t)pl * pstride + (size_t)k * total + i);
        f32x4 t[3][6];
#pragma unroll
        for (int b = 0; b < 6; ++b)
#pragma unroll
            for (int r = 0; r < 3; ++r) {
                f32x4 acc = {0.f, 0.f, 0.f, 0.f};
#pragma unroll
                for (int a = 0; a < 6; ++a) acc += W4_G[a][r] * z[a][b];
                t[r][b] = acc;
            }
        float flat[36];
#pragma unroll
        for (int r = 0; r < 3; ++r)
#pragma unroll
            for (int s2 = 0; s2 < 3; ++s2) {
                f32x4 acc = {0.f, 0.f, 0.f, 0.f};
#pragma unroll
                for (int b = 0; b < 6; ++b) acc += t[r][b] * W4_G[b][s2];
#pragma unroll
                for (int e = 0; e < 4; ++e) flat[e * 9 + r * 3 + s2] = acc[e];
            }
        f32x4* o = reinterpret_cast<f32x4*>(dw + i * 9);
#pragma unroll
        for (int j = 0; j < 9; ++j) o[j] = f32x4{flat[4 * j], flat[4 * j + 1], flat[4 * j + 2], flat[4 * j + 3]};
    }
}

int g_fused = -1;
int g_full = -1;
inline bool use_full(int mo, int K, int Nout) {
    if (mo != 4 || (K != 64 && K != 128) || g_full == 0 || g_fused == 0) return false;
    return g_full == 1;
}
int g_wino_x3 = -1;
inline bool use_x3(int mo, int K) {
    if (g_wino_x3 < 0) {
        const char* e = getenv("SSD_WINO_X3");
        g_wino_x3 = (e != nullptr && e[0] == '0') ? 0 : 1;
    }
    return g_wino_x3 == 1 && mo == 4 && K >= 256 && K % 32 == 0;
}
inline size_t align256(size_t v) { return (v + 255) & ~(size_t)255; }
inline bool use_fused(int mo, int K, int Nout) {
    if (mo != 4 || (K != 64 && K != 128 && K != 256) || g_fused == 0 || use_x3(mo, K)) return false;
    if (g_fused == 1) return true;
    return K <= 128;
}
int g_xform_cap = 8192;
inline int grid_for(size_t total) {
    const size_t b = (total + 255) / 256, cap = (size_t)g_xform_cap;
    return (int)(b > cap ? cap : (b == 0 ? 1 : b));
}

struct LatPlan { Lat lat; int TH, TW; };
LatPlan lat_plan(int H, int W, int D) {
    LatPlan p{};
    p.lat.D = D;
    int th = 0, tw = 0;
    for (int a = 0; a < 4; ++a) {
        p.lat.h0[a] = th;
        p.lat.w0[a] = tw;
        if (a < D) {
            const int sh = a < H ? (H - a + D - 1) / D : 0, sw = a < W ? (W - a + D - 1) / D : 0;
            th += (sh + 3) / 4;
            tw += (sw + 3) / 4;
        }
    }
    p.TH = th; p.TW = tw;
    return p;
}

void launch_dy_pass(const float* dy, float* Y, const ssd_conv_geom* g, int ldy, const LatPlan& lp, float* part, int bias_blocks, float* Vd,
                    const PoolSrc* ps, hipStream_t st) {
    const int TH = lp.TH, TW = lp.TW;
    const size_t tiles = (size_t)g->N * TH * TW;
    const PoolSrc none{nullptr, nullptr, 0, 0};
    if (bias_blocks > 0) {
        if (ps) hipLaunchKernelGGL((wino4_dy_kernel<true, true>), dim3(bias_blocks), dim3(256), 0, st, dy, Y, g->N, g->H, g->W, ldy, TH, TW, part, g->Co, Vd, *ps, lp.lat);
        else hipLaunchKernelGGL((wino4_dy_kernel<true, false>), dim3(bias_blocks), dim3(256), 0, st, dy, Y, g->N, g->H, g->W, ldy, TH, TW, part, g->Co, Vd, none, lp.lat);
    } else {
        const dim3 grid(grid_for(tiles * (ldy / 4)));
        if (ps) hipLaunchKernelGGL((wino4_dy_kernel<false, true>), grid, dim3(256), 0, st, dy, Y, g->N, g->H, g->W, ldy, TH, TW, static_cast<float*>(nullptr), 0, Vd, *ps, lp.lat);
        else hipLaunchKernelGGL((wino4_dy_kernel<false, false>), grid, dim3(256), 0, st, dy, Y, g->N, g->H, g->W, ldy, TH, TW, static_cast<float*>(nullptr), 0, Vd, none, lp.lat);
    }
}

struct PooledOut { float* y; uint8_t* argmax; int Ho, Wo; };
int wino_conv(int mo, const float* in, int Cin, const float* U, int U_rows, float* out, int ldo, int Cout, const float* bias,
              const float* mask, int relu, int accumulate, int N, int H, int W, void* ws, size_t ws_bytes, hipStream_t st,
              const PooledOut* pooled = nullptr, float* V_keep = nullptr, const float* V_given = nullptr,
              unsigned long long* bits_out = nullptr, const unsigned long long* mask_bits = nullptr, int D = 1) {
    if (D < 1 || D > 4 || (D > 1 && (mo != 4 || pooled != nullptr))) return SSD_ERR_BAD_SHAPE;
    const LatPlan lp = lat_plan(H, W, D);
    const int TH = mo == 4 ? lp.TH : (H + mo - 1) / mo, TW = mo == 4 ? lp.TW : (W + mo - 1) / mo, P = (mo + 2) * (mo + 2);
    const size_t tiles = (size_t)N * TH * TW;
    const int Cvalid = Cout;
    Cout = (Cout + 3) / 4 * 4;
    if (tiles >= (1ull << 31) || Cin % 32 != 0 || Cout > ldo) return SSD_ERR_BAD_SHAPE;
    const size_t vb = align256((size_t)P * tiles * Cin * 4), mb = align256((size_t)P * tiles * Cout * 4);
    if (ws_bytes < vb + mb) return SSD_ERR_WORKSPACE;
    float* V = V_keep != nullptr ? V_keep : static_cast<float*>(ws);
    float* Mx = reinterpret_cast<float*>(static_cast<char*>(ws) + vb);
    if (D == 1 && V_given == nullptr && use_full(mo, Cin, Cout))
        return ssd_internal_wino4_full(in, U, (int)tiles, Cin, U_rows, Cout, out, ldo, Cvalid, bias, mask, mask_bits, relu, accumulate, H, W, TH,
                                       TW, pooled ? pooled->y : nullptr, pooled ? pooled->argmax : nullptr, pooled ? pooled->Ho : 0,
                                       pooled ? pooled->Wo : 0, V_keep, bits_out, st);
    if (V_given != nullptr) V = const_cast<float*>(V_given);
    else if (mo == 2) hipLaunchKernelGGL(wino_input_kernel, dim3(grid_for(tiles * (Cin / 4))), dim3(256), 0, st, in, V, N, H, W, Cin, TH, TW);
    else hipLaunchKernelGGL(wino4_input_kernel, dim3(grid_for(tiles * (Cin / 4))), dim3(256), 0, st, in, V, N, H, W, Cin, TH, TW, bits_out, lp.lat);
    SSD_CHECK_LAUNCH();
    if (mask_bits != nullptr && mo != 4) return SSD_ERR_BAD_SHAPE;
    if (D == 1 && use_fused(mo, Cin, Cout))
        return ssd_internal_wino4_gemm_out(V, U, (int)tiles, Cin, U_rows, Cout, out, ldo, Cvalid, bias, mask, mask_bits, relu, accumulate, H, W, TH, TW,
                                           pooled ? pooled->y : nullptr, pooled ? pooled->argmax : nullptr, pooled ? pooled->Ho : 0,
                                           pooled ? pooled->Wo : 0, st);
    if (use_x3(mo, Cin)) {
        if (int e = ssd_internal_gemm_batched_x3(V, U, Mx, (int)tiles, Cin, Cout, U_rows, P, tiles * Cin, st)) return e;
    } else if (int e = ssd_internal_gemm_batched(V, U, Mx, (int)tiles, Cin, Cout, U_rows, P, tiles * Cin, (size_t)U_rows * Cin, 1, st)) {
        return e;
    }
    if (pooled != nullptr)
        hipLaunchKernelGGL(wino4_output_pool_kernel, dim3(grid_for(tiles * (Cout / 4))), dim3(256), 0, st, Mx, pooled->y, pooled->argmax, N, H, W,
                           Cout, TH, TW, bias, pooled->Ho, pooled->Wo);
    else if (mo == 2)
        hipLaunchKernelGGL(wino_output_kernel, dim3(grid_for(tiles * (Cout / 4))), dim3(256), 0, st, Mx, out, N, H, W, Cout, Cvalid, ldo, TH, TW,
                           bias, mask, relu, accumulate);
    else
        hipLaunchKernelGGL(wino4_output_kernel, dim3(grid_for(tiles * (Cout / 4))), dim3(256), 0, st, Mx, out, N, H, W, Cout, Cvalid, ldo, TH,
                           TW, bias, mask, relu, accumulate, mask_bits, lp.lat);
    SSD_CHECK_LAUNCH();
    return SSD_OK;
}

bool wino_geom_ok(const ssd_conv_geom* g) {
    return g && g->R == 3 && g->S == 3 && g->stride == 1 && g->dil >= 1 && g->dil <= 4 && g->pad == g->dil && g->Ho == g->H && g->Wo == g->W && g->N > 0 &&
           g->H > 0 && g->W > 0 && g->Ci > 0 && g->Co > 0;
}

}

extern "C" int ssd_wino_weights(const float* w_oihw, float* U_fwd, float* U_bwd, int Co, int Ci, int Co_pad, int mo, void* stream) {
    if (!w_oihw || (!U_fwd && !U_bwd)) return SSD_ERR_NULL;
    if (Co <= 0 || Ci <= 0 || Co_pad < Co || (mo != 2 && mo != 4)) return SSD_ERR_BAD_SHAPE;
    hipStream_t st = (hipStream_t)stream;
    if (U_fwd) {
        if (mo == 2) hipLaunchKernelGGL(wino_weight_kernel, dim3(grid_for((size_t)Co * Ci)), dim3(256), 0, st, w_oihw, U_fwd, Co, Ci, Co, Ci, 0);
        else hipLaunchKernelGGL(wino4_weight_kernel, dim3(grid_for((size_t)Co * Ci)), dim3(256), 0, st, w_oihw, U_fwd, Co, Ci, Co, Ci, 0, (int)use_x3(4, Ci));
        SSD_CHECK_LAUNCH();
    }
    if (U_bwd) {
        if (mo == 2) hipLaunchKernelGGL(wino_weight_kernel, dim3(grid_for((size_t)Ci * Co_pad)), dim3(256), 0, st, w_oihw, U_bwd, Co, Ci, Ci, Co_pad, 1);
        else hipLaunchKernelGGL(wino4_weight_kernel, dim3(grid_for((size_t)Ci * Co_pad)), dim3(256), 0, st, w_oihw, U_bwd, Co, Ci, Ci, Co_pad, 1, (int)use_x3(4, Co_pad));
        SSD_CHECK_LAUNCH();
    }
    return SSD_OK;
}

extern "C" size_t ssd_conv3x3_wino_workspace(const ssd_conv_geom* g, int direction, int mo) {
    if (!wino_geom_ok(g) || (mo != 2 && mo != 4)) return 0;
// ... 69 lines not shown
    if (ldy < g->Co || ldy % 4 != 0) return SSD_ERR_BAD_SHAPE;
    return wino_conv(4, nullptr, g->Ci, U_fwd, g->Co, y, ldy, g->Co, bias, nullptr, relu, 0, g->N, g->H, g->W, workspace, workspace_bytes,
                     (hipStream_t)stream, nullptr, nullptr, planes);
}

extern "C" int ssd_conv3x3_wino_dgrad(const float* dy, int ldy, const float* U_bwd, int Co_pad, float* dx, const float* relu_mask,
                                      int accumulate, const ssd_conv_geom* g, int mo, void* workspace, size_t workspace_bytes,
                                      void* stream) {
    if (!dy || !U_bwd || !dx || !workspace) return SSD_ERR_NULL;
    if (!wino_geom_ok(g) || Co_pad % 32 != 0 || Co_pad < g->Co || ldy != Co_pad || g->Ci % 4 != 0 || (mo != 2 && mo != 4))
        return SSD_ERR_BAD_SHAPE;
    if (!ssd_aligned16(dy) || !ssd_aligned16(dx) || !ssd_aligned16(workspace) || !ssd_aligned16(U_bwd) ||
        (relu_mask && !ssd_aligned16(relu_mask)))
        return SSD_ERR_ALIGN;
    return wino_conv(mo, dy, Co_pad, U_bwd, g->Ci, dx, g->Ci, g->Ci, nullptr, relu_mask, 0, accumulate, g->N, g->H, g->W, workspace,
                     workspace_bytes, (hipStream_t)stream, nullptr, nullptr, nullptr, nullptr, nullptr, g->dil);
}

namespace {
constexpr int COLSUM_BLOCKS = 512;
constexpr int DY_BIAS_BLOCKS = 2048;
int g_wgrad_tn = 1;
struct WinoWgradPlan { int TH, TW, Tpad, ks, cdy, P, x3; size_t tiles, yb, vb, zb, pb; LatPlan lp; };
inline bool use_x3_tn(const ssd_conv_geom* g, int mo) {
    return use_x3(mo, 256) && g_wgrad_tn && g->Co >= 128 && g->Ci >= 128 && (g->Co + 127) / 128 * 128 * 4 <= g->Co * 5 &&
           (g->Ci + 127) / 128 * 128 * 4 <= g->Ci * 5;
}
WinoWgradPlan wino_wgrad_plan(const ssd_conv_geom* g, int ldy, int mo) {
    WinoWgradPlan w;
    w.x3 = use_x3_tn(g, mo) ? 1 : 0;
    w.P = (mo + 2) * (mo + 2);
    w.lp = lat_plan(g->H, g->W, mo == 4 ? g->dil : 1);
    w.TH = mo == 4 ? w.lp.TH : (g->H + mo - 1) / mo; w.TW = mo == 4 ? w.lp.TW : (g->W + mo - 1) / mo;
    w.tiles = (size_t)g->N * w.TH * w.TW;
    w.Tpad = (int)((w.tiles + 31) / 32 * 32);
    w.cdy = ldy;
    const int bp = ((g->Co + 63) / 64) * ((g->Ci + 63) / 64) * w.P;
    int ks = (1536 + bp - 1) / bp;
    const int ksteps = w.Tpad / 32;
    if (ks > ksteps / 8) ks = ksteps / 8;
    if (ks < 1) ks = 1;
    int per = (ksteps + ks - 1) / ks;
    w.ks = (ksteps + per - 1) / per;
    if (bp > w.P && mo == 4 && (w.ks & 1) && ksteps >= 2 * (w.ks + 1)) {
        per = (ksteps + w.ks) / (w.ks + 1);
        const int k2 = (ksteps + per - 1) / per;
        if ((k2 & 1) == 0) w.ks = k2;
    }
    if (w.x3) {
        const int bp128 = ((g->Co + 127) / 128) * ((g->Ci + 127) / 128) * w.P, steps16 = (int)((w.tiles + 15) / 16);
        int k3 = 768 / bp128;
        if (k3 > 1) k3 &= ~1;
        if (k3 > steps16 / 8) k3 = steps16 / 8;
        if (k3 < 1) k3 = 1;
        const int per3 = (steps16 + k3 - 1) / k3;
        w.ks = (steps16 + per3 - 1) / per3;
    }
    w.yb = align256((size_t)w.P * ldy * w.Tpad * 4);
    w.vb = align256((size_t)w.P * g->Ci * w.Tpad * 4);
    w.zb = align256((size_t)w.P * w.ks * g->Co * g->Ci * 4);
    w.pb = align256((size_t)DY_BIAS_BLOCKS * ldy * 4);
    return w;
}
int launch_wgrad_tn(const float* Y, const float* V, float* Zs, const ssd_conv_geom* g, int ldy, const WinoWgradPlan& w, hipStream_t st) {
    if (w.x3) {
        const int steps16 = (int)((w.tiles + 15) / 16);
        return ssd_internal_gemm_tn_x3(Y, V, Zs, g->Co, g->Ci, (int)w.tiles, ldy, g->Ci, w.P, w.ks, (steps16 + w.ks - 1) / w.ks, w.tiles * ldy,
                                       w.tiles * g->Ci, st);
    }
    TnParams q;
    q.a = Y; q.b = V; q.out = Zs;
    q.M = g->Co; q.N = g->Ci; q.K = (int)w.tiles; q.lda = ldy; q.ldb = g->Ci;
    q.tiles_m = (g->Co + 63) / 64; q.tiles_n = (g->Ci + 63) / 64;
    const int ksteps = (q.K + 31) / 32;
    q.ksplit = w.ks;
    q.ksteps_per_split = (ksteps + w.ks - 1) / w.ks;
    q.batch_a = w.tiles * ldy; q.batch_b = w.tiles * g->Ci;
    if (q.batch_a * 4 >= 0xFFFFFFF0ull || q.batch_b * 4 >= 0xFFFFFFF0ull) return SSD_ERR_BAD_SHAPE;
    q.a_bytes = (unsigned)(q.batch_a * 4); q.b_bytes = (unsigned)(q.batch_b * 4);
    q.groups = w.P * w.ks;
    hipLaunchKernelGGL(wino_gemm_tn_kernel, dim3((unsigned)(q.tiles_m * q.tiles_n * ((q.groups + 7) / 8) * 8)), dim3(256), 0, st, q);
    SSD_CHECK_LAUNCH();
    return SSD_OK;
}
}

extern "C" int ssd_tune_set_wino_x3(int on) {
    g_wino_x3 = on < 0 ? -1 : (on != 0);
    return SSD_OK;
}
extern "C" int ssd_wino_uses_x3(int mo, int K) { return use_x3(mo, K) ? 1 : 0; }

extern "C" int ssd_tune_set_wino_bias_tail(int on) {
    g_bias_tail = on != 0;
    return SSD_OK;
}
extern "C" int ssd_tune_set_wino_xform_blocks(int blocks) {
    if (blocks < 64 || blocks > 65535) return SSD_ERR_BAD_SHAPE;
    g_xform_cap = blocks;
    return SSD_OK;
}

extern "C" int ssd_tune_set_wino_full(int mode) {
    if (mode < -1 || mode > 1) return SSD_ERR_BAD_SHAPE;
#ifndef SSD_EXPERIMENTAL
    if (mode == 1) return SSD_ERR_BAD_SHAPE;
#endif
    g_full = mode;
    return SSD_OK;
}

extern "C" int ssd_conv3x3_wino_uses_full(const ssd_conv_geom* g, int direction) {
    if (!wino_geom_ok(g) || g->dil != 1) return 0;
    const int co_pad = (g->Co + 31) / 32 * 32;
    return direction == 0 ? use_full(4, g->Ci, (g->Co + 3) / 4 * 4) : use_full(4, co_pad, g->Ci);
}

extern "C" int ssd_tune_set_wino_fused(int mode) {
    if (mode < -1 || mode > 1) return SSD_ERR_BAD_SHAPE;
    g_fused = mode;
    return SSD_OK;
}

extern "C" int ssd_tune_set_wino_wgrad_tn(int on) {
    g_wgrad_tn = on ? 1 : 0;
    return SSD_OK;
}

extern "C" size_t ssd_conv3x3_wino_wgrad_workspace(const ssd_conv_geom* g, int ldy, int mo) {
    if (!wino_geom_ok(g) || ldy < g->Co || (mo != 2 && mo != 4)) return 0;
    const WinoWgradPlan w = wino_wgrad_plan(g, ldy, mo);
    return w.yb + w.vb + w.zb + w.pb;
}

namespace {
int wino_wgrad(const float* x, const float* planes, const float* dy, int ldy, float* dw_oihw, float* dbias, const ssd_conv_geom* g, int mo,
               float* dgrad_planes, void* workspace, size_t workspace_bytes, void* stream, const PoolSrc* pool = nullptr);
}
extern "C" int ssd_conv3x3_wino_wgrad(const float* x, const float* dy, int ldy, float* dw_oihw, float* dbias, const ssd_conv_geom* g,
                                      int mo, void* workspace, size_t workspace_bytes, void* stream) {
    if (!x) return SSD_ERR_NULL;
    if (!ssd_aligned16(x)) return SSD_ERR_ALIGN;
    return wino_wgrad(x, nullptr, dy, ldy, dw_oihw, dbias, g, mo, nullptr, workspace, workspace_bytes, stream);
}
extern "C" int ssd_conv3x3_wino_wgrad_planes(const float* planes, const float* dy, int ldy, float* dw_oihw, float* dbias,
                                             const ssd_conv_geom* g, float* dgrad_planes_out, void* workspace, size_t workspace_bytes,
                                             void* stream) {
    if (!planes) return SSD_ERR_NULL;
    if (!ssd_aligned16(planes) || (dgrad_planes_out && !ssd_aligned16(dgrad_planes_out))) return SSD_ERR_ALIGN;
    return wino_wgrad(nullptr, planes, dy, ldy, dw_oihw, dbias, g, 4, dgrad_planes_out, workspace, workspace_bytes, stream);
}
extern "C" int ssd_conv3x3_wino_dgrad_bits(const float* dy, int ldy, const float* U_bwd, int Co_pad, float* dx, const uint64_t* relu_bits,
                                           int accumulate, const ssd_conv_geom* g, void* workspace, size_t workspace_bytes, void* stream) {
    if (!dy || !U_bwd || !dx || !workspace || !relu_bits) return SSD_ERR_NULL;
    if (!wino_geom_ok(g) || Co_pad % 32 != 0 || Co_pad < g->Co || ldy != Co_pad || g->Ci % 4 != 0) return SSD_ERR_BAD_SHAPE;
    if (!ssd_aligned16(dy) || !ssd_aligned16(dx) || !ssd_aligned16(workspace) || !ssd_aligned16(U_bwd) || ((uintptr_t)relu_bits & 7))
        return SSD_ERR_ALIGN;
    return wino_conv(4, dy, Co_pad, U_bwd, g->Ci, dx, g->Ci, g->Ci, nullptr, nullptr, 0, accumulate, g->N, g->H, g->W, workspace, workspace_bytes,
                     (hipStream_t)stream, nullptr, nullptr, nullptr, nullptr, reinterpret_cast<const unsigned long long*>(relu_bits), g->dil);
}
extern "C" int ssd_conv3x3_wino_dgrad_planes_bits(const float* dy_planes, const float* U_bwd, int Co_pad, float* dx, const uint64_t* relu_bits,
                                                  int accumulate, const ssd_conv_geom* g, void* workspace, size_t workspace_bytes,
                                                  void* stream) {
    if (!dy_planes || !U_bwd || !dx || !workspace || !relu_bits) return SSD_ERR_NULL;
    if (!wino_geom_ok(g) || Co_pad % 32 != 0 || Co_pad < g->Co || g->Ci % 4 != 0) return SSD_ERR_BAD_SHAPE;
    if (!ssd_aligned16(dy_planes) || !ssd_aligned16(dx) || !ssd_aligned16(workspace) || !ssd_aligned16(U_bwd) || ((uintptr_t)relu_bits & 7))
        return SSD_ERR_ALIGN;
    return wino_conv(4, nullptr, Co_pad, U_bwd, g->Ci, dx, g->Ci, g->Ci, nullptr, nullptr, 0, accumulate, g->N, g->H, g->W, workspace,
                     workspace_bytes, (hipStream_t)stream, nullptr, nullptr, dy_planes, nullptr,
                     reinterpret_cast<const unsigned long long*>(relu_bits), g->dil);
}
extern "C" int ssd_conv3x3_wino_dgrad_planes(const float* dy_planes, const float* U_bwd, int Co_pad, float* dx, const float* relu_mask,
                                             int accumulate, const ssd_conv_geom* g, void* workspace, size_t workspace_bytes, void* stream) {
    if (!dy_planes || !U_bwd || !dx || !workspace) return SSD_ERR_NULL;
    if (!wino_geom_ok(g) || Co_pad % 32 != 0 || Co_pad < g->Co || g->Ci % 4 != 0) return SSD_ERR_BAD_SHAPE;
    if (!ssd_aligned16(dy_planes) || !ssd_aligned16(dx) || !ssd_aligned16(workspace) || !ssd_aligned16(U_bwd) ||
        (relu_mask && !ssd_aligned16(relu_mask)))
        return SSD_ERR_ALIGN;
    return wino_conv(4, nullptr, Co_pad, U_bwd, g->Ci, dx, g->Ci, g->Ci, nullptr, relu_mask, 0, accumulate, g->N, g->H, g->W, workspace,
                     workspace_bytes, (hipStream_t)stream, nullptr, nullptr, dy_planes, nullptr, nullptr, g->dil);
}
namespace {
int wino_wgrad(const float* x, const float* planes, const float* dy, int ldy, float* dw_oihw, float* dbias, const ssd_conv_geom* g, int mo,
               float* dgrad_planes, void* workspace, size_t workspace_bytes, void* stream, const PoolSrc* pool) {
    if (!dy || !dw_oihw || !workspace) return SSD_ERR_NULL;
    if (!wino_geom_ok(g) || g->Ci % 4 != 0 || ldy % 4 != 0 || ldy < g->Co || (mo != 2 && mo != 4)) return SSD_ERR_BAD_SHAPE;
    if (!ssd_aligned16(dy) || !ssd_aligned16(workspace) || !ssd_aligned16(dw_oihw)) return SSD_ERR_ALIGN;
    const WinoWgradPlan w = wino_wgrad_plan(g, ldy, mo);
    if (w.tiles >= (1ull << 31)) return SSD_ERR_BAD_SHAPE;
    if (workspace_bytes < w.yb + w.vb + w.zb + w.pb) return SSD_ERR_WORKSPACE;
    hipStream_t st = (hipStream_t)stream;
    char* base = static_cast<char*>(workspace);
    float* Yt = reinterpret_cast<float*>(base);
    float* Vt = reinterpret_cast<float*>(base + w.yb);
    float* Zs = reinterpret_cast<float*>(base + w.yb + w.vb);
    float* part = reinterpret_cast<float*>(base + w.yb + w.vb + w.zb);
    const int gy = (w.Tpad / 32) * ((ldy / 4 + 7) / 8), gx = (w.Tpad / 32) * ((g->Ci / 4 + 7) / 8);
    const dim3 gyd(gy > 16384 ? 16384 : gy), gxd(gx > 16384 ? 16384 : gx);
    int dy_bias_blocks = 0;
    if (dgrad_planes != nullptr && !(mo == 4 && (g_wgrad_tn || planes != nullptr))) return SSD_ERR_BAD_SHAPE;
    if (g->dil != 1 && (pool != nullptr || !(mo == 4 && (g_wgrad_tn || planes != nullptr)))) return SSD_ERR_BAD_SHAPE;
    if (mo == 4 && (g_wgrad_tn || planes != nullptr)) {
        const int c4 = ldy / 4;
        if (dbias != nullptr && c4 <= 256) {
            int gcd = 256, r = c4;
            while (r) { const int tmp = gcd % r; gcd = r; r = tmp; }
            const int unit = c4 / gcd;
            int blocks = grid_for(w.tiles * c4);
            if (blocks > DY_BIAS_BLOCKS) blocks = DY_BIAS_BLOCKS;
            blocks = (blocks + unit - 1) / unit * unit;
            if (blocks > DY_BIAS_BLOCKS) blocks -= unit;
            dy_bias_blocks = blocks;
            launch_dy_pass(dy, Yt, g, ldy, w.lp, part, blocks, dgrad_planes, pool, st);
        } else
            launch_dy_pass(dy, Yt, g, ldy, w.lp, nullptr, 0, dgrad_planes, pool, st);
        if (planes == nullptr)
            hipLaunchKernelGGL(wino4_input_kernel, dim3(grid_for(w.tiles * (g->Ci / 4))), dim3(256), 0, st, x, Vt, g->N, g->H, g->W, g->Ci, w.TH,
                               w.TW, static_cast<unsigned long long*>(nullptr), w.lp.lat);
        SSD_CHECK_LAUNCH();
        if (int e = launch_wgrad_tn(Yt, planes != nullptr ? planes : Vt, Zs, g, ldy, w, st)) return e;
    } else if (mo == 2) {
        hipLaunchKernelGGL(wino_xform_t_kernel<1>, gyd, dim3(256), 0, st, dy, Yt, g->N, g->H, g->W, ldy, w.TH, w.TW, w.Tpad);
        hipLaunchKernelGGL(wino_xform_t_kernel<0>, gxd, dim3(256), 0, st, x, Vt, g->N, g->H, g->W, g->Ci, w.TH, w.TW, w.Tpad);
    } else {
        hipLaunchKernelGGL(wino4_xform_t_kernel<1>, gyd, dim3(256), 0, st, dy, Yt, g->N, g->H, g->W, ldy, w.TH, w.TW, w.Tpad);
        hipLaunchKernelGGL(wino4_xform_t_kernel<0>, gxd, dim3(256), 0, st, x, Vt, g->N, g->H, g->W, g->Ci, w.TH, w.TW, w.Tpad);
    }
    SSD_CHECK_LAUNCH();
    if (!(mo == 4 && (g_wgrad_tn || planes != nullptr)))
        if (int e = ssd_internal_gemm_batched(Yt, Vt, Zs, g->Co, w.Tpad, g->Ci, g->Ci, w.P, (size_t)ldy * w.Tpad, (size_t)g->Ci * w.Tpad, w.ks, st))
            return e;
    if (mo == 2)
        hipLaunchKernelGGL(wino_wgrad_finish_kernel, dim3(grid_for((size_t)g->Co * g->Ci)), dim3(256), 0, st, Zs, dw_oihw, g->Co, g->Ci, w.ks);
    else
    {
        const size_t total = (size_t)g->Co * g->Ci;
        int ks_left = w.ks;
        if (w.ks > 1 && total / 4 < 65536) {
            hipLaunchKernelGGL(wino_splitk_sum_kernel, dim3(grid_for(total / 4 * w.P)), dim3(256), 0, st, Zs, total, w.P, w.ks);
            SSD_CHECK_LAUNCH();
            ks_left = 1;
        }
        const int nfin = grid_for(total / 4), ldp = (g->Co + 3) / 4 * 4;
        const bool tail = dbias && dy_bias_blocks > 0 && g_bias_tail;
        const BiasTail bt{tail ? part : nullptr, dbias, dy_bias_blocks, g->Co, ldp};
        hipLaunchKernelGGL(wino4_wgrad_finish_kernel, dim3(nfin + (tail ? (ldp + 15) / 16 : 0)), dim3(256), 0, st, Zs, dw_oihw, g->Co, g->Ci,
                           ks_left, (size_t)w.ks * total, nfin, bt);
    }
    SSD_CHECK_LAUNCH();
    if (dbias && dy_bias_blocks > 0 && !g_bias_tail) {
        const int ldp = (g->Co + 3) / 4 * 4;
        hipLaunchKernelGGL(colsum_final4_kernel, dim3((ldp + 15) / 16), dim3(256), 0, st, part, dbias, dy_bias_blocks, g->Co, ldp);
        SSD_CHECK_LAUNCH();
    }
    if (dbias && dy_bias_blocks == 0) {
        const size_t M = (size_t)g->N * g->H * g->W;
        int cq = 1;
        while (cq < (g->Co + 3) / 4 && cq < 256) cq <<= 1;
        hipLaunchKernelGGL(colsum_partial_kernel, dim3(COLSUM_BLOCKS), dim3(256), 0, st, dy, part, M, ldy, g->Co, cq);
        SSD_CHECK_LAUNCH();
        hipLaunchKernelGGL(colsum_final_kernel, dim3((g->Co + 15) / 16), dim3(256), 0, st, part, dbias, COLSUM_BLOCKS, g->Co);
        SSD_CHECK_LAUNCH();
    }
    return SSD_OK;
}
}


namespace {
int dy_bias_blocks_for(const ssd_conv_geom* g, int ldy, size_t tiles) {
    const int c4 = ldy / 4;
    if (c4 > 256) return 0;
    int gcd = 256, r = c4;
    while (r) { const int tmp = gcd % r; gcd = r; r = tmp; }
    const int unit = c4 / gcd;
    int blocks = grid_for(tiles * c4);
    if (blocks > DY_BIAS_BLOCKS) blocks = DY_BIAS_BLOCKS;
    blocks = (blocks + unit - 1) / unit * unit;
    if (blocks > DY_BIAS_BLOCKS) blocks -= unit;
    if (blocks < unit) blocks = unit;
    return blocks;
}
}

extern "C" size_t ssd_wino4_bias_partial_floats(const ssd_conv_geom* g, int ldy) {
    if (!wino_geom_ok(g) || ldy < g->Co || ldy % 4 != 0) return 0;
    return (size_t)DY_BIAS_BLOCKS * ldy;
}

namespace {
int dy_transform(const float* dy, int ldy, const ssd_conv_geom* g, float* wgrad_planes, float* dgrad_planes_out, float* bias_partial,
                 const PoolSrc* pool, void* stream) {
    if (!dy || !wgrad_planes) return SSD_ERR_NULL;
    if (!wino_geom_ok(g) || ldy % 4 != 0 || ldy < g->Co) return SSD_ERR_BAD_SHAPE;
    if (!ssd_aligned16(dy) || !ssd_aligned16(wgrad_planes) || (dgrad_planes_out && !ssd_aligned16(dgrad_planes_out)) ||
        (bias_partial && !ssd_aligned16(bias_partial)))
        return SSD_ERR_ALIGN;
    if (pool != nullptr && g->dil != 1) return SSD_ERR_BAD_SHAPE;
    const LatPlan lp = lat_plan(g->H, g->W, g->dil);
    const size_t tiles = (size_t)g->N * lp.TH * lp.TW;
    if (tiles >= (1ull << 31)) return SSD_ERR_BAD_SHAPE;
    hipStream_t st = (hipStream_t)stream;
    const int blocks = bias_partial ? dy_bias_blocks_for(g, ldy, tiles) : 0;
    if (bias_partial && blocks == 0) return SSD_ERR_BAD_SHAPE;
    launch_dy_pass(dy, wgrad_planes, g, ldy, lp, bias_partial, blocks, dgrad_planes_out, pool, st);
    SSD_CHECK_LAUNCH();
    return SSD_OK;
}
}

extern "C" int ssd_wino4_dy_transform(const float* dy, int ldy, const ssd_conv_geom* g, float* wgrad_planes, float* dgrad_planes_out,
                                      float* bias_partial, void* stream) {
    return dy_transform(dy, ldy, g, wgrad_planes, dgrad_planes_out, bias_partial, nullptr, stream);
}

namespace {
int pool_src(const ssd_conv_geom* g, int ldy, const float* dpool, const unsigned char* argmax, const float* y_pooled, int Hp, int Wp, PoolSrc* ps) {
    if (!dpool || !argmax || !y_pooled) return SSD_ERR_NULL;
    if (!wino_geom_ok(g) || g->dil != 1 || ldy != g->Co || Hp < g->H / 2 || Wp < g->W / 2 || Hp <= 0 || Wp <= 0 || 2 * Hp > g->H + 1 || 2 * Wp > g->W + 1)
        return SSD_ERR_BAD_SHAPE;
    if (!ssd_aligned16(y_pooled) || ((uintptr_t)argmax & 3) != 0) return SSD_ERR_ALIGN;
    ps->am = argmax; ps->gate = y_pooled; ps->Hp = Hp; ps->Wp = Wp;
    return SSD_OK;
}
}

extern "C" int ssd_wino4_dy_transform_pooled(const float* dpool, const unsigned char* argmax, const float* y_pooled, int Hp, int Wp, int ldy,
                                             const ssd_conv_geom* g, float* wgrad_planes, float* dgrad_planes_out, float* bias_partial,
                                             void* stream) {
    if (!g) return SSD_ERR_NULL;
    PoolSrc ps;
    const int e = pool_src(g, ldy, dpool, argmax, y_pooled, Hp, Wp, &ps);
    return e != SSD_OK ? e : dy_transform(dpool, ldy, g, wgrad_planes, dgrad_planes_out, bias_partial, &ps, stream);
}

extern "C" int ssd_conv3x3_wino_wgrad_planes_pooled(const float* planes, const float* dpool, const unsigned char* argmax, const float* y_pooled,
                                                    int Hp, int Wp, int ldy, float* dw_oihw, float* dbias, const ssd_conv_geom* g,
                                                    float* dgrad_planes_out, void* workspace, size_t workspace_bytes, void* stream) {
    if (!planes || !g) return SSD_ERR_NULL;
    if (!ssd_aligned16(planes) || (dgrad_planes_out && !ssd_aligned16(dgrad_planes_out))) return SSD_ERR_ALIGN;
    PoolSrc ps;
    const int e = pool_src(g, ldy, dpool, argmax, y_pooled, Hp, Wp, &ps);
    return e != SSD_OK ? e : wino_wgrad(nullptr, planes, dpool, ldy, dw_oihw, dbias, g, 4, dgrad_planes_out, workspace, workspace_bytes, stream, &ps);
}

extern "C" size_t ssd_wino4_wgrad_gemm_workspace(const ssd_conv_geom* g, int ldy) {
    if (!wino_geom_ok(g) || ldy < g->Co) return 0;
    return wino_wgrad_plan(g, ldy, 4).zb;
}

extern "C" int ssd_wino4_wgrad_gemm(const float* wgrad_planes, const float* x_planes, int ldy, const float* bias_partial, float* dw_oihw,
                                    float* dbias, const ssd_conv_geom* g, void* workspace, size_t workspace_bytes, void* stream) {
    if (!wgrad_planes || !x_planes || !dw_oihw || !workspace) return SSD_ERR_NULL;
    if (!wino_geom_ok(g) || g->Ci % 4 != 0 || ldy % 4 != 0 || ldy < g->Co) return SSD_ERR_BAD_SHAPE;
    if (dbias && !bias_partial) return SSD_ERR_NULL;
    if (!ssd_aligned16(wgrad_planes) || !ssd_aligned16(x_planes) || !ssd_aligned16(dw_oihw) || !ssd_aligned16(workspace)) return SSD_ERR_ALIGN;
    const WinoWgradPlan w = wino_wgrad_plan(g, ldy, 4);
    if (workspace_bytes < w.zb) return SSD_ERR_WORKSPACE;
    hipStream_t st = (hipStream_t)stream;
    float* Zs = static_cast<float*>(workspace);
    if (int e = launch_wgrad_tn(wgrad_planes, x_planes, Zs, g, ldy, w, st)) return e;
    const size_t total = (size_t)g->Co * g->Ci;
    int ks_left = w.ks;
    if (w.ks > 1 && total / 4 < 65536) {
        hipLaunchKernelGGL(wino_splitk_sum_kernel, dim3(grid_for(total / 4 * w.P)), dim3(256), 0, st, Zs, total, w.P, w.ks);
        SSD_CHECK_LAUNCH();
        ks_left = 1;
    }
    const int blocks = dbias ? dy_bias_blocks_for(g, ldy, w.tiles) : 0;
    if (dbias && blocks == 0) return SSD_ERR_BAD_SHAPE;
    const int nfin = grid_for(total / 4), ldp = (g->Co + 3) / 4 * 4;
    const BiasTail bt{dbias ? bias_partial : nullptr, dbias, blocks, g->Co, ldp};
    hipLaunchKernelGGL(wino4_wgrad_finish_kernel, dim3(nfin + (dbias ? (ldp + 15) / 16 : 0)), dim3(256), 0, st, Zs, dw_oihw, g->Co, g->Ci, ks_left,
                       (size_t)w.ks * total, nfin, bt);
    SSD_CHECK_LAUNCH();
    return SSD_OK;
}

extern "C" int ssd_wino_weights_adj(const float* w_oihw, float* U_adj, int Co, int Ci, int Co_pad, void* stream) {
    if (!w_oihw || !U_adj) return SSD_ERR_NULL;
    if (Co <= 0 || Ci <= 0 || Co_pad < Co) return SSD_ERR_BAD_SHAPE;
    hipLaunchKernelGGL(wino4_weight_kernel, dim3(grid_for((size_t)Ci * Co_pad)), dim3(256), 0, (hipStream_t)stream, w_oihw, U_adj, Co, Ci, Ci, Co_pad, 2,
                       (int)use_x3(4, Co_pad));
    SSD_CHECK_LAUNCH();
    return SSD_OK;
}

extern "C" size_t ssd_wino4_adj_planes_floats(const ssd_conv_geom* g) {
    if (!wino_geom_ok(g) || g->dil != 1) return 0;
    const LatPlan lp = lat_plan(g->H, g->W, 1);
    return (size_t)36 * g->N * lp.TH * lp.TW * ((g->Ci + 3) / 4 * 4);
}

extern "C" int ssd_conv3x3_wino_dgrad_adj_gemm(const float* y_planes, int ldy, const float* U_adj, float* md_planes, const ssd_conv_geom* g,
                                               void* stream) {
    if (!y_planes || !U_adj || !md_planes) return SSD_ERR_NULL;
    if (!wino_geom_ok(g) || g->dil != 1 || ldy % 32 != 0 || ldy < g->Co || g->Ci % 4 != 0) return SSD_ERR_BAD_SHAPE;
    if (!ssd_aligned16(y_planes) || !ssd_aligned16(U_adj) || !ssd_aligned16(md_planes)) return SSD_ERR_ALIGN;
    const LatPlan lp = lat_plan(g->H, g->W, 1);
    const size_t tiles = (size_t)g->N * lp.TH * lp.TW;
    if (tiles >= (1ull << 31)) return SSD_ERR_BAD_SHAPE;
    hipStream_t st = (hipStream_t)stream;
    if (use_x3(4, ldy)) return ssd_internal_gemm_batched_x3(y_planes, U_adj, md_planes, (int)tiles, ldy, g->Ci, g->Ci, 36, tiles * ldy, st);
    return ssd_internal_gemm_batched(y_planes, U_adj, md_planes, (int)tiles, ldy, g->Ci, g->Ci, 36, tiles * ldy, (size_t)g->Ci * ldy, 1, st);
}

extern "C" int ssd_wino4_adj_output(const float* md_planes, float* dx, const float* relu_mask, const uint64_t* relu_bits, int accumulate,
                                    const ssd_conv_geom* g, void* stream) {
    if (!md_planes || !dx) return SSD_ERR_NULL;
    if (!wino_geom_ok(g) || g->dil != 1 || g->Ci % 4 != 0) return SSD_ERR_BAD_SHAPE;
    if (!ssd_aligned16(md_planes) || !ssd_aligned16(dx) || (relu_mask && !ssd_aligned16(relu_mask)) || (relu_bits && ((uintptr_t)relu_bits & 7)))
        return SSD_ERR_ALIGN;
    const LatPlan lp = lat_plan(g->H, g->W, 1);
    const size_t tiles = (size_t)g->N * lp.TH * lp.TW;
    hipLaunchKernelGGL((wino4_adj_out_kernel<false, false>), dim3(grid_for(tiles * (g->Ci / 4))), dim3(256), 0, (hipStream_t)stream, md_planes, g->N, g->H,
                       g->W, g->Ci, lp.TH, lp.TW, dx, g->Ci, relu_mask, reinterpret_cast<const unsigned long long*>(relu_bits), accumulate,
                       static_cast<float*>(nullptr), static_cast<float*>(nullptr), 0);
    SSD_CHECK_LAUNCH();
    return SSD_OK;
}

extern "C" int ssd_wino4_adj_output_to_planes(const float* md_planes, const float* relu_mask, const uint64_t* relu_bits, const ssd_conv_geom* g,
                                              const ssd_conv_geom* g_below, float* y_planes, float* bias_partial, void* stream) {
    if (!md_planes || !y_planes || !g_below) return SSD_ERR_NULL;
    if (!wino_geom_ok(g) || !wino_geom_ok(g_below) || g->dil != 1 || g_below->dil != 1 || g->Ci % 4 != 0 || g_below->Co != g->Ci ||
        g_below->N != g->N || g_below->H != g->H || g_below->W != g->W)
        return SSD_ERR_BAD_SHAPE;
    if (!ssd_aligned16(md_planes) || !ssd_aligned16(y_planes) || (relu_mask && !ssd_aligned16(relu_mask)) || (relu_bits && ((uintptr_t)relu_bits & 7)) ||
        (bias_partial && !ssd_aligned16(bias_partial)))
        return SSD_ERR_ALIGN;
    const LatPlan lp = lat_plan(g->H, g->W, 1);
    const size_t tiles = (size_t)g->N * lp.TH * lp.TW;
    hipStream_t st = (hipStream_t)stream;
    if (bias_partial) {
        const int blocks = dy_bias_blocks_for(g_below, g->Ci, tiles);
        if (blocks == 0) return SSD_ERR_BAD_SHAPE;
        hipLaunchKernelGGL((wino4_adj_out_kernel<true, true>), dim3(blocks), dim3(256), 0, st, md_planes, g->N, g->H, g->W, g->Ci, lp.TH, lp.TW,
                           static_cast<float*>(nullptr), g->Ci, relu_mask, reinterpret_cast<const unsigned long long*>(relu_bits), 0, y_planes, bias_partial,
                           g_below->Co);
    } else {
        hipLaunchKernelGGL((wino4_adj_out_kernel<true, false>), dim3(grid_for(tiles * (g->Ci / 4))), dim3(256), 0, st, md_planes, g->N, g->H, g->W, g->Ci,
                           lp.TH, lp.TW, static_cast<float*>(nullptr), g->Ci, relu_mask, reinterpret_cast<const unsigned long long*>(relu_bits), 0, y_planes,
                           static_cast<float*>(nullptr), 0);
    }
    SSD_CHECK_LAUNCH();
    return SSD_OK;
}

namespace {
__global__ __launch_bounds__(256) void weight_jobs_kernel(const ssd_weight_job* __restrict__ jobs, const int* __restrict__ block_start, int njobs) {
    int lo = 0, hi = njobs - 1;
    while (lo < hi) {
        const int mid = (lo + hi + 1) >> 1;
        if (block_start[mid] <= (int)blockIdx.x) lo = mid; else hi = mid - 1;
    }
    const ssd_weight_job j = jobs[lo];
    const size_t i = (size_t)((int)blockIdx.x - block_start[lo]) * 256 + threadIdx.x;
// ... 170 lines not shown
```

objectdetection_ssd_amd/ops.py:

```python
from __future__ import annotations

import contextlib
import ctypes as C
from typing import List, Optional, Tuple

import torch

from . import _lib
from ._lib import ConvGeom, check


def _stream() -> int:
    return torch.cuda.current_stream().cuda_stream


_current_device = torch.cuda.current_device


def _req(t: torch.Tensor, name: str, dtype=torch.float32) -> torch.Tensor:
    if not isinstance(t, torch.Tensor):
        raise TypeError(f"{name}: expected a tensor")
    if not t.is_cuda:
        raise RuntimeError(f"{name}: the gfx950 path needs a device tensor (got {t.device}); there is no CPU fallback")
    if t.device.index != _current_device():
# ... 1238 lines not shown
        raise ValueError("conv2d_fwd_wino_pool: not a 3x3 / stride 1 / pad 1 geometry")
    ws = workspace(nbytes, x.device, "wino")
    planes = wino_planes(g, x.device) if keep_planes else None
    bits = wino_relu_bits(g, x.device) if want_bits else None
    check(lib.ssd_conv3x3_wino_fwd_pool_bits(x.data_ptr(), u_fwd.data_ptr(), _ptr(bias), y.data_ptr(), _ptr(am), C.byref(g), int(ceil_mode),
                                             _ptr(planes), _ptr(bits), ws.data_ptr(), ws.numel(), _stream()), "conv2d_fwd_wino_pool")
    if want_bits:
        return y, am, planes, bits
    return (y, am, planes) if keep_planes else (y, am)


def conv2d_fwd_wino_from_planes(planes: torch.Tensor, u_fwd: torch.Tensor, bias: Optional[torch.Tensor], g: ConvGeom, relu: bool = True,
                                pool_ceil: Optional[bool] = None, want_argmax: bool = True):
    _req(planes, "planes")
    if _wino_mo(u_fwd) != 4 or tuple(planes.shape) != tuple(wino_planes_shape(g)) or g.Co % 4 != 0:
        raise ValueError("conv2d_fwd_wino_from_planes: planes / filters do not match the geometry")
    _wino_filter(u_fwd, "u_fwd", g.Co, g.Ci)
    if bias is not None:
        _req(bias, "bias")
    lib = _lib.load()
    nbytes = lib.ssd_conv3x3_wino_workspace(C.byref(g), 0, 4)
    if nbytes == 0:
        raise ValueError("conv2d_fwd_wino_from_planes: not a 3x3 / stride 1 / pad 1 geometry")
    ws = workspace(nbytes, planes.device, "wino")
    if pool_ceil is None:
        y = torch.empty((g.N, g.H, g.W, g.Co), device=planes.device, dtype=torch.float32)
        check(lib.ssd_conv3x3_wino_fwd_from_planes(planes.data_ptr(), u_fwd.data_ptr(), _ptr(bias), y.data_ptr(), g.Co, None, None, C.byref(g), int(relu),
                                                   0, ws.data_ptr(), ws.numel(), _stream()), "conv2d_fwd_wino_from_planes")
        return y
    ho, wo = pool_out(g.H, 2, 2, 0, pool_ceil), pool_out(g.W, 2, 2, 0, pool_ceil)
    y = torch.empty((g.N, ho, wo, g.Co), device=planes.device, dtype=torch.float32)
    am = torch.empty((g.N, ho, wo, g.Co), device=planes.device, dtype=torch.uint8) if want_argmax else None
    check(lib.ssd_conv3x3_wino_fwd_from_planes(planes.data_ptr(), u_fwd.data_ptr(), _ptr(bias), None, 0, y.data_ptr(), _ptr(am), C.byref(g), 1,
                                               int(pool_ceil), ws.data_ptr(), ws.numel(), _stream()), "conv2d_fwd_wino_from_planes")
    return y, am


def conv2d_dgrad_wino(dy: Optional[torch.Tensor], u_bwd: torch.Tensor, g: ConvGeom, dx: Optional[torch.Tensor] = None,
                      relu_mask: Optional[torch.Tensor] = None, accumulate: bool = False,
                      planes: Optional[torch.Tensor] = None, bits: Optional[torch.Tensor] = None) -> torch.Tensor:
    mo = _wino_mo(u_bwd)
    co_pad = _wino_filter(u_bwd, "u_bwd", g.Ci, None)
    dev = u_bwd.device
    if planes is not None:
        _req(planes, "planes")
        if mo != 4 or tuple(planes.shape) != (36, wino_planes_shape(g)[1], co_pad):
            raise ValueError("conv2d_dgrad_wino: planes do not match the geometry")
    else:
        _req(dy, "dy")
        if dy.numel() != g.N * g.H * g.W * co_pad:
            raise ValueError("conv2d_dgrad_wino: shapes do not match the geometry")
    if dx is None:
        if accumulate:
            raise ValueError("accumulate needs an existing dx")
        dx = torch.empty((g.N, g.H, g.W, g.Ci), device=dev, dtype=torch.float32)
    _req(dx, "dx")
    if relu_mask is not None:
        _req(relu_mask, "relu_mask")
    lib = _lib.load()
    ws = workspace(lib.ssd_conv3x3_wino_workspace(C.byref(g), 1, mo), dev, "wino")
    if bits is not None:
        _req(bits, "bits", torch.int64)
        if mo != 4 or tuple(bits.shape) != (wino_planes_shape(g)[1], g.Ci // 4) or g.Ci % 4 != 0:
            raise ValueError("conv2d_dgrad_wino: bits need F(4x4) filters and one word per (tile, channel quad)")
        if planes is None:
            check(lib.ssd_conv3x3_wino_dgrad_bits(dy.data_ptr(), co_pad, u_bwd.data_ptr(), co_pad, dx.data_ptr(), bits.data_ptr(), int(accumulate),
                                                  C.byref(g), ws.data_ptr(), ws.numel(), _stream()), "conv2d_dgrad_wino")
            return dx
        check(lib.ssd_conv3x3_wino_dgrad_planes_bits(planes.data_ptr(), u_bwd.data_ptr(), co_pad, dx.data_ptr(), bits.data_ptr(), int(accumulate),
                                                     C.byref(g), ws.data_ptr(), ws.numel(), _stream()), "conv2d_dgrad_wino")
        return dx
    if planes is not None:
        check(lib.ssd_conv3x3_wino_dgrad_planes(planes.data_ptr(), u_bwd.data_ptr(), co_pad, dx.data_ptr(), _ptr(relu_mask), int(accumulate),
                                                C.byref(g), ws.data_ptr(), ws.numel(), _stream()), "conv2d_dgrad_wino")
        return dx
    check(lib.ssd_conv3x3_wino_dgrad(dy.data_ptr(), co_pad, u_bwd.data_ptr(), co_pad, dx.data_ptr(), _ptr(relu_mask), int(accumulate),
                                     C.byref(g), mo, ws.data_ptr(), ws.numel(), _stream()), "conv2d_dgrad_wino")
    return dx


def conv2d_wgrad_wino(x: Optional[torch.Tensor], dy: torch.Tensor, g: ConvGeom, ldy: int, want_bias: bool = True, mo: int = 2,
                      planes: Optional[torch.Tensor] = None, dgrad_planes: bool = False,
                      dw_out: Optional[torch.Tensor] = None, db_out: Optional[torch.Tensor] = None):
    pooled = isinstance(dy, PooledGrad)
    if pooled and planes is None:
        raise ValueError("conv2d_wgrad_wino: a pooled gradient needs the kept forward planes")
    if not pooled:
        _req(dy, "dy")
    if planes is not None:
        _req(planes, "planes")
        if mo != 4 or tuple(planes.shape) != tuple(wino_planes_shape(g)):
            raise ValueError("conv2d_wgrad_wino: planes do not match the geometry")
    else:
        _req(x, "x")
        if tuple(x.shape) != (g.N, g.H, g.W, g.Ci):
            raise ValueError("conv2d_wgrad_wino: shapes do not match the geometry")
    if not pooled and dy.numel() != g.N * g.H * g.W * ldy:
        raise ValueError("conv2d_wgrad_wino: shapes do not match the geometry")
    lib = _lib.load()
    nbytes = lib.ssd_conv3x3_wino_wgrad_workspace(C.byref(g), ldy, mo)
    if nbytes == 0:
        raise ValueError("conv2d_wgrad_wino: not a 3x3 / stride 1 / pad 1 geometry")
    dev = planes.device if pooled else dy.device
    ws = workspace(nbytes, dev, "wino")
    dw = _grad_dst(dw_out, (g.Co, g.Ci, 3, 3), dev, "dw_out")
    db = _grad_dst(db_out, (g.Co,), dev, "db_out") if want_bias else None
    if dgrad_planes and planes is None:
        raise ValueError("conv2d_wgrad_wino: dgrad_planes needs the kept forward planes")
    if planes is not None:
        pd = torch.empty((36, planes.shape[1], ldy), device=dev, dtype=torch.float32) if dgrad_planes else None
        if pooled:
            check(lib.ssd_conv3x3_wino_wgrad_planes_pooled(planes.data_ptr(), *_pooled_args(dy, g, ldy), ldy, dw.data_ptr(), _ptr(db), C.byref(g),
                                                           _ptr(pd), ws.data_ptr(), ws.numel(), _stream()), "conv2d_wgrad_wino_pooled")
            return (dw, db, pd) if dgrad_planes else (dw, db)
        check(lib.ssd_conv3x3_wino_wgrad_planes(planes.data_ptr(), dy.data_ptr(), ldy, dw.data_ptr(), _ptr(db), C.byref(g), _ptr(pd),
                                                ws.data_ptr(), ws.numel(), _stream()), "conv2d_wgrad_wino")
        return (dw, db, pd) if dgrad_planes else (dw, db)
    check(lib.ssd_conv3x3_wino_wgrad(x.data_ptr(), dy.data_ptr(), ldy, dw.data_ptr(), _ptr(db), C.byref(g), mo, ws.data_ptr(), ws.numel(),
                                     _stream()), "conv2d_wgrad_wino")
    return dw, db


def wino_dy_transform(dy: torch.Tensor, g: ConvGeom, ldy: int, dgrad_planes: bool = True, want_bias: bool = True):
    pooled = isinstance(dy, PooledGrad)
    dev = dy.dpool.device if pooled else _req(dy, "dy").device
    tiles = wino_planes_shape(g)[1]
    if (not pooled and dy.numel() != g.N * g.H * g.W * ldy) or ldy % 4 != 0 or ldy < g.Co:
        raise ValueError("wino_dy_transform: shapes do not match the geometry")
    lib = _lib.load()
    Y = torch.empty((36, tiles, ldy), device=dev, dtype=torch.float32)
    Vd = torch.empty((36, tiles, ldy), device=dev, dtype=torch.float32) if dgrad_planes else None
    part = torch.empty((lib.ssd_wino4_bias_partial_floats(C.byref(g), ldy),), device=dev, dtype=torch.float32) if want_bias else None
    if pooled:
        check(lib.ssd_wino4_dy_transform_pooled(*_pooled_args(dy, g, ldy), ldy, C.byref(g), Y.data_ptr(), _ptr(Vd), _ptr(part), _stream()),
              "wino_dy_transform_pooled")
    else:
        check(lib.ssd_wino4_dy_transform(dy.data_ptr(), ldy, C.byref(g), Y.data_ptr(), _ptr(Vd), _ptr(part), _stream()), "wino_dy_transform")
    return Y, Vd, part


def wino_adj_weights(w_oihw: torch.Tensor, co_pad: int) -> torch.Tensor:
    _req(w_oihw, "w")
    co, ci = int(w_oihw.shape[0]), int(w_oihw.shape[1])
    u = wino_filter_alloc(4, ci, co_pad, w_oihw.device)
    check(_lib.load().ssd_wino_weights_adj(w_oihw.data_ptr(), u.data_ptr(), co, ci, co_pad, _stream()), "wino_weights_adj")
    return u


def wino_dgrad_adj_gemm(y_planes: torch.Tensor, u_adj: torch.Tensor, g: ConvGeom, ldy: int) -> torch.Tensor:
    _req(y_planes, "y_planes")
    tiles = wino_planes_shape(g)[1]
    if tuple(y_planes.shape) != (36, tiles, ldy) or g.Ci % 4 != 0 or ldy % 32 != 0:
        raise ValueError("wino_dgrad_adj_gemm: planes do not match the geometry")
    _wino_filter(u_adj, "u_adj", g.Ci, ldy)
    md = torch.empty((36, tiles, g.Ci), device=y_planes.device, dtype=torch.float32)
    check(_lib.load().ssd_conv3x3_wino_dgrad_adj_gemm(y_planes.data_ptr(), ldy, u_adj.data_ptr(), md.data_ptr(), C.byref(g), _stream()),
          "wino_dgrad_adj_gemm")
    return md


def _adj_mask_args(g: ConvGeom, tiles: int, relu_mask, bits):
    if bits is not None:
        _req(bits, "bits", torch.int64)
        if tuple(bits.shape) != (tiles, g.Ci // 4):
            raise ValueError("adjoint output: one mask word per (tile, channel quad)")
    if relu_mask is not None:
        _req(relu_mask, "relu_mask")
        if relu_mask.numel() != g.N * g.H * g.W * g.Ci:
            raise ValueError("adjoint output: relu_mask must have dx's shape")


def wino_adj_output(md: torch.Tensor, g: ConvGeom, dx: Optional[torch.Tensor] = None, relu_mask: Optional[torch.Tensor] = None,
                    bits: Optional[torch.Tensor] = None, accumulate: bool = False) -> torch.Tensor:
    _req(md, "md")
    tiles = wino_planes_shape(g)[1]
    if tuple(md.shape) != (36, tiles, g.Ci):
        raise ValueError("wino_adj_output: planes do not match the geometry")
    _adj_mask_args(g, tiles, relu_mask, bits)
    if dx is None:
        if accumulate:
            raise ValueError("accumulate needs an existing dx")
        dx = torch.empty((g.N, g.H, g.W, g.Ci), device=md.device, dtype=torch.float32)
    _req(dx, "dx")
    if dx.numel() != g.N * g.H * g.W * g.Ci:
        raise ValueError("wino_adj_output: dx shape")
    check(_lib.load().ssd_wino4_adj_output(md.data_ptr(), dx.data_ptr(), _ptr(relu_mask) if bits is None else None, _ptr(bits), int(accumulate),
                                           C.byref(g), _stream()), "wino_adj_output")
    return dx


def wino_adj_output_to_planes(md: torch.Tensor, g: ConvGeom, g_below: ConvGeom, relu_mask: Optional[torch.Tensor] = None,
                              bits: Optional[torch.Tensor] = None, want_bias: bool = True):
    _req(md, "md")
    tiles = wino_planes_shape(g)[1]
    if tuple(md.shape) != (36, tiles, g.Ci) or g_below.Co != g.Ci or (g_below.N, g_below.H, g_below.W) != (g.N, g.H, g.W):
        raise ValueError("wino_adj_output_to_planes: the two layers do not chain")
    _adj_mask_args(g, tiles, relu_mask, bits)
    lib = _lib.load()
    Y = torch.empty((36, tiles, g.Ci), device=md.device, dtype=torch.float32)
    part = torch.empty((lib.ssd_wino4_bias_partial_floats(C.byref(g_below), g.Ci),), device=md.device, dtype=torch.float32) if want_bias else None
    check(lib.ssd_wino4_adj_output_to_planes(md.data_ptr(), _ptr(relu_mask) if bits is None else None, _ptr(bits), C.byref(g), C.byref(g_below),
                                             Y.data_ptr(), _ptr(part), _stream()), "wino_adj_output_to_planes")
    return Y, part


class AdjPlanesGrad:

    def __init__(self, md: torch.Tensor, g: ConvGeom, relu_mask: Optional[torch.Tensor], bits: Optional[torch.Tensor]):
        self.md, self.g, self.relu_mask, self.bits = md, g, relu_mask, bits

    @property
    def shape(self):
        return (self.g.N, self.g.H, self.g.W, self.g.Ci)

    def materialize(self) -> torch.Tensor:
        return wino_adj_output(self.md, self.g, None, self.relu_mask, self.bits, False)


class PooledGrad:

    def __init__(self, dpool: torch.Tensor, argmax: torch.Tensor, y_pooled: torch.Tensor, in_shape):
        _req(dpool, "dpool"); _req(y_pooled, "y_pooled"); _req(argmax, "argmax", torch.uint8)
        if tuple(dpool.shape) != tuple(y_pooled.shape) or tuple(argmax.shape) != tuple(dpool.shape) or dpool.shape[3] != in_shape[3]:
            raise ValueError("PooledGrad: dpool, argmax and the pooled output must have one shape, and the channels of the pool's input")
        self.dpool, self.argmax, self.y_pooled, self.in_shape = dpool, argmax, y_pooled, tuple(in_shape)

    def materialize(self, dx: Optional[torch.Tensor] = None) -> torch.Tensor:
        return maxpool_bwd(self.dpool, self.argmax, self.in_shape, 2, 2, 0, dx, y_gate=self.y_pooled)


def _pooled_args(dy: "PooledGrad", g: ConvGeom, ldy: int):
    if dy.in_shape != (g.N, g.H, g.W, g.Co) or ldy != g.Co:
        raise ValueError("pooled gradient does not match the geometry")
    return dy.dpool.data_ptr(), dy.argmax.data_ptr(), dy.y_pooled.data_ptr(), dy.dpool.shape[1], dy.dpool.shape[2]


def wino_wgrad_gemm(wgrad_planes: torch.Tensor, x_planes: torch.Tensor, bias_partial: Optional[torch.Tensor], g: ConvGeom, ldy: int,
                    dw_out: Optional[torch.Tensor] = None, db_out: Optional[torch.Tensor] = None):
    _req(wgrad_planes, "wgrad_planes"); _req(x_planes, "x_planes")
    tiles = wino_planes_shape(g)[1]
    if tuple(wgrad_planes.shape) != (36, tiles, ldy) or tuple(x_planes.shape) != (36, tiles, g.Ci):
        raise ValueError("wino_wgrad_gemm: planes do not match the geometry")
    lib = _lib.load()
    dev = x_planes.device
    ws = workspace(lib.ssd_wino4_wgrad_gemm_workspace(C.byref(g), ldy), dev, "wino_wgrad")
    dw = _grad_dst(dw_out, (g.Co, g.Ci, 3, 3), dev, "dw_out")
    db = _grad_dst(db_out, (g.Co,), dev, "db_out") if bias_partial is not None else None
    check(lib.ssd_wino4_wgrad_gemm(wgrad_planes.data_ptr(), x_planes.data_ptr(), ldy, _ptr(bias_partial), dw.data_ptr(), _ptr(db), C.byref(g),
                                   ws.data_ptr(), ws.numel(), _stream()), "wino_wgrad_gemm")
    return dw, db


class WeightTable:

    def __init__(self, jobs, device):
        import numpy as np
        lib = _lib.load()
        arr = (_lib.WeightJob * len(jobs))()
        starts, total = [], 0
        self.keep = []
        for a, j in zip(arr, jobs):
            for t in (j["w0"], j.get("w1"), j.get("out_fwd"), j.get("out_bwd")):
                if t is not None:
                    _req(t, "weight job tensor", t.dtype if (j["kind"] in (0, 3, 4) and t.dtype == torch.bfloat16) else torch.float32)
                    self.keep.append(t)
            a.w0 = j["w0"].data_ptr()
            a.w1 = j["w1"].data_ptr() if j.get("w1") is not None else j["w0"].data_ptr()
            a.out_fwd = _ptr(j.get("out_fwd"))
            a.out_bwd = _ptr(j.get("out_bwd"))
            a.co0, a.co, a.ci, a.taps, a.co_pad, a.kind = j["co0"], j["co"], j["ci"], j["taps"], j["co_pad"], j["kind"]
            a.pad1 = j.get("pad1", 0)
            if j["kind"] == 0:
                a.pad0 = sum(bit for bit, key in ((1, "out_fwd"), (2, "out_bwd")) if j.get(key) is not None and j[key].dtype == torch.bfloat16)
                if j.get("adj"):
                    a.pad0 |= 4
            nb = lib.ssd_weight_job_blocks(C.byref(a))
            if nb <= 0:
                raise ValueError("bad weight job")
            starts.append(total)
            total += nb
        self.njobs, self.total_blocks = len(jobs), total
        self.jobs_dev = torch.from_numpy(np.frombuffer(bytes(arr), dtype=np.uint8).copy()).to(device)
        self.starts_dev = torch.tensor(starts, dtype=torch.int32).to(device)

    def run(self) -> None:
        check(_lib.load().ssd_weights_prepare(self.jobs_dev.data_ptr(), self.starts_dev.data_ptr(), self.njobs, self.total_blocks, _stream()),
              "weights_prepare")
```

Baseline: 1615.

## Fuse accumulating maxpool backward into Winograd dy transform and restructure wgrad finish

Adds a lazy pooled gradient that carries a base gradient and a full-resolution ReLU mask. The Winograd dy-transform can then fold the max-unpool scatter, the accumulation into the base and the mask into one pass, instead of materialising the accumulated gradient first. It also merges the split-K sum into the wgrad finish kernel using 576-thread blocks that stage partial sums in shared memory, removing a separate launch and round trip. The column-sum bias kernels get 8-way unrolled loads for more memory-level parallelism. The trade-offs are added complexity and extra fallback paths that materialise when shapes do not match.

```diff
diff --git a/include/ssd_gfx950.h b/include/ssd_gfx950.h
--- a/include/ssd_gfx950.h
+++ b/include/ssd_gfx950.h
@@ -130,6 +130,9 @@
                          const ssd_conv_geom* g, void* workspace, size_t workspace_bytes, void* stream);
 int ssd_wino4_dy_transform_pooled(const float* dpool, const unsigned char* argmax, const float* y_pooled, int Hp, int Wp, int ldy,
                                   const ssd_conv_geom* g, float* wgrad_planes, float* dgrad_planes_out, float* bias_partial, void* stream);
+int ssd_wino4_dy_transform_pooled_base(const float* dpool, const unsigned char* argmax, const float* base, const float* mask, int Hp, int Wp,
+                                       int ldy, const ssd_conv_geom* g, float* wgrad_planes, float* dgrad_planes_out, float* bias_partial,
+                                       void* stream);
 int ssd_conv3x3_wino_wgrad_planes_pooled(const float* planes, const float* dpool, const unsigned char* argmax, const float* y_pooled,
                                          int Hp, int Wp, int ldy, float* dw_oihw, float* dbias, const ssd_conv_geom* g,
                                          float* dgrad_planes_out, void* workspace, size_t workspace_bytes, void* stream);
diff --git a/objectdetection_ssd_amd/Model.py b/objectdetection_ssd_amd/Model.py
--- a/objectdetection_ssd_amd/Model.py
+++ b/objectdetection_ssd_amd/Model.py
@@ -779,6 +779,8 @@
                        and not ops.wino_uses_full(g, 1))
                 if isinstance(dy, ops.AdjPlanesGrad) and not adj:
                     dy = dy.materialize()
+                if isinstance(dy, ops.PooledGrad) and dy.base is not None and not adj:
+                    dy = dy.materialize()
                 if adj:
                     name = op["p"]
                     kept = aux.pop("planes:" + name)
@@ -903,6 +905,11 @@
                     ops.PooledGrad(dy, am, yout, xin.shape)
                     if (self.lazy_pool_grad and isinstance(xin, _Elided) and mask is not None and not acc and dx is None
                         and (op["k"], op["s"], op["pad"]) == (2, 2, 0)) else
+                    ops.PooledGrad(dy, am, None, xin.shape, base=dx, mask=mask)
+                    if (self.lazy_pool_grad and acc and dx is not None and torch.is_tensor(mask) and torch.is_tensor(xin)
+                        and dy.dtype == torch.float32 and dx.dtype == torch.float32 and mask.dtype == torch.float32
+                        and (op["k"], op["s"], op["pad"]) == (2, 2, 0) and xin.shape[1] % 2 == 0 and xin.shape[2] % 2 == 0
+                        and self.grad_tap is None and self._conv_of.get(op["x"]) is not None) else
                     ops.maxpool_bwd(dy, am, tuple(xin.shape), op["k"], op["s"], op["pad"], dx, y_gate=yout)
                     if (mask is not None and not acc) else
                     ops.maxpool_bwd(dy, am, tuple(xin.shape), op["k"], op["s"], op["pad"], dx, mask, acc)))
diff --git a/objectdetection_ssd_amd/_lib.py b/objectdetection_ssd_amd/_lib.py
--- a/objectdetection_ssd_amd/_lib.py
+++ b/objectdetection_ssd_amd/_lib.py
@@ -134,6 +134,7 @@
     "ssd_wino4_adj_output": (_I, [_P, _P, _P, _P, _I, _G, _P]),
     "ssd_wino4_adj_output_to_planes": (_I, [_P, _P, _P, _G, _G, _P, _P, _P]),
     "ssd_wino4_dy_transform_pooled": (_I, [_P, _P, _P, _I, _I, _I, _G, _P, _P, _P, _P]),
+    "ssd_wino4_dy_transform_pooled_base": (_I, [_P, _P, _P, _P, _I, _I, _I, _G, _P, _P, _P, _P]),
     "ssd_conv3x3_wino_wgrad_planes_pooled": (_I, [_P, _P, _P, _P, _I, _I, _I, _P, _P, _G, _P, _P, _Z, _P]),
     "ssd_wino4_wgrad_gemm_workspace": (_Z, [_G, _I]),
     "ssd_wino4_wgrad_gemm": (_I, [_P, _P, _I, _P, _P, _P, _G, _P, _Z, _P]),
diff --git a/objectdetection_ssd_amd/csrc/gemm_x3.hip b/objectdetection_ssd_amd/csrc/gemm_x3.hip
--- a/objectdetection_ssd_amd/csrc/gemm_x3.hip
+++ b/objectdetection_ssd_amd/csrc/gemm_x3.hip
@@ -820,9 +820,19 @@
 }
 __global__ __launch_bounds__(256) void x3_colsum_partial_kernel(const float* __restrict__ dy, float* __restrict__ part, size_t M, int ld) {
     const int q4 = ld >> 2;
+    const size_t G = gridDim.x;
     for (int q = threadIdx.x; q < q4; q += 256) {
+        const float* col = dy + q * 4;
         f32x4 s0 = {0.f, 0.f, 0.f, 0.f};
-        for (size_t m = blockIdx.x; m < M; m += gridDim.x) s0 += *reinterpret_cast<const f32x4*>(dy + m * ld + q * 4);
+        size_t m = blockIdx.x;
+        for (; m + 7 * G < M; m += 8 * G) {
+            f32x4 v[8];
+#pragma unroll
+            for (int j = 0; j < 8; ++j) v[j] = *reinterpret_cast<const f32x4*>(col + (m + j * G) * ld);
+#pragma unroll
+            for (int j = 0; j < 8; ++j) s0 += v[j];
+        }
+        for (; m < M; m += G) s0 += *reinterpret_cast<const f32x4*>(col + m * ld);
         *reinterpret_cast<f32x4*>(part + (size_t)blockIdx.x * ld + q * 4) = s0;
     }
 }
@@ -831,8 +841,17 @@
     const int cl = threadIdx.x & 63, q = threadIdx.x >> 6;
     const int c = blockIdx.x * 64 + cl;
     float t = 0.f;
-    if (c < C)
-        for (int k = q; k < nblk; k += 4) t += part[(size_t)k * ld + c];
+    if (c < C) {
+        int k = q;
+        for (; k + 28 < nblk; k += 32) {
+            float v[8];
+#pragma unroll
+            for (int j = 0; j < 8; ++j) v[j] = part[(size_t)(k + 4 * j) * ld + c];
+#pragma unroll
+            for (int j = 0; j < 8; ++j) t += v[j];
+        }
+        for (; k < nblk; k += 4) t += part[(size_t)k * ld + c];
+    }
     red[q][cl] = t;
     __syncthreads();
     if (q == 0 && c < C) db[c] = ((red[0][cl] + red[1][cl]) + red[2][cl]) + red[3][cl];
diff --git a/objectdetection_ssd_amd/csrc/winograd.hip b/objectdetection_ssd_amd/csrc/winograd.hip
--- a/objectdetection_ssd_amd/csrc/winograd.hip
+++ b/objectdetection_ssd_amd/csrc/winograd.hip
@@ -1,4 +1,5 @@
 #include <cstdlib>
+#include <type_traits>
 #include "common.h"
 
 int ssd_internal_gemm_batched(const float* a, const float* w, float* out, int M, int K, int N, int n_rows, int nbatch,
@@ -629,8 +630,8 @@
     }
 }
 
-struct PoolSrc { const uint8_t* am; const float* gate; int Hp, Wp; };
-template <bool BIAS, bool POOLED = false>
+struct PoolSrc { const uint8_t* am; const float* gate; int Hp, Wp; const float* base; const float* mask; };
+template <bool BIAS, bool POOLED = false, bool BASE = false>
 __global__ __launch_bounds__(256) void wino4_dy_kernel(const float* __restrict__ dy, float* __restrict__ Y, int N, int H, int W, int C,
                                                        int TH, int TW, float* __restrict__ part, int Cvalid, float* __restrict__ Vd,
                                                        const PoolSrc ps, const Lat lat) {
@@ -660,10 +661,13 @@
                     if (ok) {
                         const size_t idx = (((size_t)n * ps.Hp + ph) * ps.Wp + pw) * C4 + c4;
                         d = *reinterpret_cast<const f32x4*>(dy + idx * 4);
-                        const f32x4 yv = *reinterpret_cast<const f32x4*>(ps.gate + idx * 4);
-                        a = *reinterpret_cast<const uint32_t*>(ps.am + idx * 4);
-#pragma unroll
-                        for (int e = 0; e < 4; ++e) d[e] = yv[e] > 0.f ? d[e] : 0.f;
+                        if (!BASE) {
+                            const f32x4 yv = *reinterpret_cast<const f32x4*>(ps.gate + idx * 4);
+                            a = *reinterpret_cast<const uint32_t*>(ps.am + idx * 4);
+#pragma unroll
+                            for (int e = 0; e < 4; ++e) d[e] = yv[e] > 0.f ? d[e] : 0.f;
+                        } else
+                            a = *reinterpret_cast<const uint32_t*>(ps.am + idx * 4);
                     }
                     pg[r][q] = d;
                     pc[r][q] = a;
@@ -678,6 +682,21 @@
             const int r = (a + 1) >> 1, q = (b + 1) >> 1;
             const uint32_t code = (uint32_t)(((a + 1) & 1) * 2 + ((b + 1) & 1));
             f32x4 g;
+            if (BASE) {
+                g = f32x4{0.f, 0.f, 0.f, 0.f};
+                if (ok) {
+                    const size_t o = (((size_t)n * H + ih) * W + iw) * C + c4 * 4;
+                    const f32x4 bv = *reinterpret_cast<const f32x4*>(ps.base + o), mv = *reinterpret_cast<const f32x4*>(ps.mask + o);
+#pragma unroll
+                    for (int e = 0; e < 4; ++e) {
+                        float v = 0.f;
+                        if (((pc[r][q] >> (8 * e)) & 0xffu) == code) v += pg[r][q][e];
+                        v += bv[e];
+                        g[e] = mv[e] > 0.f ? v : 0.f;
+                    }
+                }
+                return g;
+            }
 #pragma unroll
             for (int e = 0; e < 4; ++e) g[e] = (ok && ((pc[r][q] >> (8 * e)) & 0xffu) == code) ? pg[r][q][e] : 0.f;
             return g;
@@ -995,21 +1014,86 @@
     }
 }
 
-__global__ __launch_bounds__(256) void wino_splitk_sum_kernel(float* __restrict__ Zs, size_t total, int P, int ksplit) {
-    const size_t quads = total >> 2, n = quads * P;
-    for (size_t idx = (size_t)blockIdx.x * 256 + threadIdx.x; idx < n; idx += (size_t)gridDim.x * 256) {
-        const size_t pl = idx / quads, q = idx - pl * quads;
-        float* src = Zs + pl * ksplit * total + q * 4;
-        f32x4 sum = *reinterpret_cast<const f32x4*>(src);
-        for (int k = 1; k < ksplit; ++k) sum += *reinterpret_cast<const f32x4*>(src + (size_t)k * total);
-        *reinterpret_cast<f32x4*>(src) = sum;
-    }
-}
-
-__global__ __launch_bounds__(256) void wino4_wgrad_finish_kernel(const float* __restrict__ Zs, float* __restrict__ dw, int Co, int Ci, int ksplit,
-                                                                 size_t pstride, int nfin, const BiasTail bt) {
+__device__ __forceinline__ void wgrad_finish_quad(const f32x4 (&z)[6][6], float* __restrict__ dw9) {
+    f32x4 t[3][6];
+#pragma unroll
+    for (int b = 0; b < 6; ++b)
+#pragma unroll
+        for (int r = 0; r < 3; ++r) {
+            f32x4 acc = {0.f, 0.f, 0.f, 0.f};
+#pragma unroll
+            for (int a = 0; a < 6; ++a) acc += W4_G[a][r] * z[a][b];
+            t[r][b] = acc;
+        }
+    float flat[36];
+#pragma unroll
+    for (int r = 0; r < 3; ++r)
+#pragma unroll
+        for (int s2 = 0; s2 < 3; ++s2) {
+            f32x4 acc = {0.f, 0.f, 0.f, 0.f};
+#pragma unroll
+            for (int b = 0; b < 6; ++b) acc += t[r][b] * W4_G[b][s2];
+#pragma unroll
+            for (int e = 0; e < 4; ++e) flat[e * 9 + r * 3 + s2] = acc[e];
+        }
+    f32x4* o = reinterpret_cast<f32x4*>(dw9);
+#pragma unroll
+    for (int j = 0; j < 9; ++j) o[j] = f32x4{flat[4 * j], flat[4 * j + 1], flat[4 * j + 2], flat[4 * j + 3]};
+}
+
+template <int QB>
+__global__ __launch_bounds__(QB ? 576 : 256) void wino4_wgrad_finish_kernel(const float* __restrict__ Zs, float* __restrict__ dw, int Co, int Ci,
+                                                                             int ksplit, size_t pstride, int nfin, const BiasTail bt) {
     if ((int)blockIdx.x >= nfin) {
+        if (QB && threadIdx.x >= 256) return;
         colsum_final4_body(bt.part, bt.db, bt.nblk, bt.C, bt.ldp, (int)blockIdx.x - nfin);
+        return;
+    }
+    if constexpr (QB != 0) {
+        constexpr int I = QB / 16, KB = 8 / I;
+        __shared__ f32x4 zl[36][QB];
+        const size_t total = (size_t)Co * Ci, quads = total >> 2, groups = (quads + QB - 1) / QB;
+        const int pl = threadIdx.x >> 4, ql = threadIdx.x & 15;
+        for (size_t gq = blockIdx.x; gq < groups; gq += (size_t)nfin) {
+            const float* src[I];
+            f32x4 sum[I];
+#pragma unroll
+            for (int i = 0; i < I; ++i) {
+                const size_t q = gq * QB + i * 16 + ql;
+                src[i] = Zs + (size_t)pl * pstride + (q < quads ? q : quads - 1) * 4;
+                sum[i] = *reinterpret_cast<const f32x4*>(src[i]);
+            }
+            int k = 1;
+            for (; k + KB <= ksplit; k += KB) {
+                f32x4 v[I][KB];
+#pragma unroll
+                for (int j = 0; j < KB; ++j)
+#pragma unroll
+                    for (int i = 0; i < I; ++i) v[i][j] = *reinterpret_cast<const f32x4*>(src[i] + (size_t)(k + j) * total);
+#pragma unroll
+                for (int j = 0; j < KB; ++j)
+#pragma unroll
+                    for (int i = 0; i < I; ++i) sum[i] += v[i][j];
+            }
+            for (; k < ksplit; ++k) {
+                f32x4 v[I];
+#pragma unroll
+                for (int i = 0; i < I; ++i) v[i] = *reinterpret_cast<const f32x4*>(src[i] + (size_t)k * total);
+#pragma unroll
+                for (int i = 0; i < I; ++i) sum[i] += v[i];
+            }
+#pragma unroll
+            for (int i = 0; i < I; ++i) zl[pl][i * 16 + ql] = sum[i];
+            __syncthreads();
+            const size_t q = gq * QB + threadIdx.x;
+            if (threadIdx.x < QB && q < quads) {
+                f32x4 z[6][6];
+#pragma unroll
+                for (int p2 = 0; p2 < 36; ++p2) z[p2 / 6][p2 % 6] = zl[p2][threadIdx.x];
+                wgrad_finish_quad(z, dw + q * 4 * 9);
+            }
+            __syncthreads();
+        }
         return;
     }
     const size_t total = (size_t)Co * Ci, quads = total >> 2;
@@ -1021,30 +1105,7 @@
         for (int k = 1; k < ksplit; ++k)
 #pragma unroll
             for (int pl = 0; pl < 36; ++pl) z[pl / 6][pl % 6] += *reinterpret_cast<const f32x4*>(Zs + (size_t)pl * pstride + (size_t)k * total + i);
-        f32x4 t[3][6];
-#pragma unroll
-        for (int b = 0; b < 6; ++b)
-#pragma unroll
-            for (int r = 0; r < 3; ++r) {
-                f32x4 acc = {0.f, 0.f, 0.f, 0.f};
-#pragma unroll
-                for (int a = 0; a < 6; ++a) acc += W4_G[a][r] * z[a][b];
-                t[r][b] = acc;
-            }
-        float flat[36];
-#pragma unroll
-        for (int r = 0; r < 3; ++r)
-#pragma unroll
-            for (int s2 = 0; s2 < 3; ++s2) {
-                f32x4 acc = {0.f, 0.f, 0.f, 0.f};
-#pragma unroll
-                for (int b = 0; b < 6; ++b) acc += t[r][b] * W4_G[b][s2];
-#pragma unroll
-                for (int e = 0; e < 4; ++e) flat[e * 9 + r * 3 + s2] = acc[e];
-            }
-        f32x4* o = reinterpret_cast<f32x4*>(dw + i * 9);
-#pragma unroll
-        for (int j = 0; j < 9; ++j) o[j] = f32x4{flat[4 * j], flat[4 * j + 1], flat[4 * j + 2], flat[4 * j + 3]};
+        wgrad_finish_quad(z, dw + i * 9);
     }
 }
 
@@ -1096,7 +1157,15 @@
                     const PoolSrc* ps, hipStream_t st) {
     const int TH = lp.TH, TW = lp.TW;
     const size_t tiles = (size_t)g->N * TH * TW;
-    const PoolSrc none{nullptr, nullptr, 0, 0};
+    const PoolSrc none{nullptr, nullptr, 0, 0, nullptr, nullptr};
+    if (ps && ps->base) {
+        if (bias_blocks > 0)
+            hipLaunchKernelGGL((wino4_dy_kernel<true, true, true>), dim3(bias_blocks), dim3(256), 0, st, dy, Y, g->N, g->H, g->W, ldy, TH, TW, part, g->Co, Vd, *ps, lp.lat);
+        else
+            hipLaunchKernelGGL((wino4_dy_kernel<false, true, true>), dim3(grid_for(tiles * (ldy / 4))), dim3(256), 0, st, dy, Y, g->N, g->H, g->W, ldy, TH, TW,
+                               static_cast<float*>(nullptr), 0, Vd, *ps, lp.lat);
+        return;
+    }
     if (bias_blocks > 0) {
         if (ps) hipLaunchKernelGGL((wino4_dy_kernel<true, true>), dim3(bias_blocks), dim3(256), 0, st, dy, Y, g->N, g->H, g->W, ldy, TH, TW, part, g->Co, Vd, *ps, lp.lat);
         else hipLaunchKernelGGL((wino4_dy_kernel<true, false>), dim3(bias_blocks), dim3(256), 0, st, dy, Y, g->N, g->H, g->W, ldy, TH, TW, part, g->Co, Vd, none, lp.lat);
@@ -1332,6 +1401,23 @@
     hipLaunchKernelGGL(wino_gemm_tn_kernel, dim3((unsigned)(q.tiles_m * q.tiles_n * ((q.groups + 7) / 8) * 8)), dim3(256), 0, st, q);
     SSD_CHECK_LAUNCH();
     return SSD_OK;
+}
+void launch_wgrad_finish(const float* Zs, float* dw_oihw, const ssd_conv_geom* g, int ks, const BiasTail& bt, hipStream_t st) {
+    const size_t total = (size_t)g->Co * g->Ci;
+    const int tail = bt.part ? (bt.ldp + 15) / 16 : 0;
+    auto slabs = [&](auto qb) {
+        constexpr int QB = decltype(qb)::value;
+        const int nfin = (int)((total / 4 + QB - 1) / QB);
+        hipLaunchKernelGGL(wino4_wgrad_finish_kernel<QB>, dim3(nfin + tail), dim3(576), 0, st, Zs, dw_oihw, g->Co, g->Ci, ks, (size_t)ks * total, nfin, bt);
+    };
+    if (ks > 1 && total / 4 < 65536) {
+        if (total / 4 >= 64 * 256) slabs(std::integral_constant<int, 64>{});
+        else if (total / 4 >= 32 * 256) slabs(std::integral_constant<int, 32>{});
+        else slabs(std::integral_constant<int, 16>{});
+    } else {
+        const int nfin = grid_for(total / 4);
+        hipLaunchKernelGGL(wino4_wgrad_finish_kernel<0>, dim3(nfin + tail), dim3(256), 0, st, Zs, dw_oihw, g->Co, g->Ci, ks, (size_t)ks * total, nfin, bt);
+    }
 }
 }
 
@@ -1484,18 +1570,9 @@
         hipLaunchKernelGGL(wino_wgrad_finish_kernel, dim3(grid_for((size_t)g->Co * g->Ci)), dim3(256), 0, st, Zs, dw_oihw, g->Co, g->Ci, w.ks);
     else
     {
-        const size_t total = (size_t)g->Co * g->Ci;
-        int ks_left = w.ks;
-        if (w.ks > 1 && total / 4 < 65536) {
-            hipLaunchKernelGGL(wino_splitk_sum_kernel, dim3(grid_for(total / 4 * w.P)), dim3(256), 0, st, Zs, total, w.P, w.ks);
-            SSD_CHECK_LAUNCH();
-            ks_left = 1;
-        }
-        const int nfin = grid_for(total / 4), ldp = (g->Co + 3) / 4 * 4;
+        const int ldp = (g->Co + 3) / 4 * 4;
         const bool tail = dbias && dy_bias_blocks > 0 && g_bias_tail;
-        const BiasTail bt{tail ? part : nullptr, dbias, dy_bias_blocks, g->Co, ldp};
-        hipLaunchKernelGGL(wino4_wgrad_finish_kernel, dim3(nfin + (tail ? (ldp + 15) / 16 : 0)), dim3(256), 0, st, Zs, dw_oihw, g->Co, g->Ci,
-                           ks_left, (size_t)w.ks * total, nfin, bt);
+        launch_wgrad_finish(Zs, dw_oihw, g, w.ks, BiasTail{tail ? part : nullptr, dbias, dy_bias_blocks, g->Co, ldp}, st);
     }
     SSD_CHECK_LAUNCH();
     if (dbias && dy_bias_blocks > 0 && !g_bias_tail) {
@@ -1570,7 +1647,7 @@
     if (!wino_geom_ok(g) || g->dil != 1 || ldy != g->Co || Hp < g->H / 2 || Wp < g->W / 2 || Hp <= 0 || Wp <= 0 || 2 * Hp > g->H + 1 || 2 * Wp > g->W + 1)
         return SSD_ERR_BAD_SHAPE;
     if (!ssd_aligned16(y_pooled) || ((uintptr_t)argmax & 3) != 0) return SSD_ERR_ALIGN;
-    ps->am = argmax; ps->gate = y_pooled; ps->Hp = Hp; ps->Wp = Wp;
+    ps->am = argmax; ps->gate = y_pooled; ps->Hp = Hp; ps->Wp = Wp; ps->base = nullptr; ps->mask = nullptr;
     return SSD_OK;
 }
 }
@@ -1582,6 +1659,19 @@
     PoolSrc ps;
     const int e = pool_src(g, ldy, dpool, argmax, y_pooled, Hp, Wp, &ps);
     return e != SSD_OK ? e : dy_transform(dpool, ldy, g, wgrad_planes, dgrad_planes_out, bias_partial, &ps, stream);
+}
+
+extern "C" int ssd_wino4_dy_transform_pooled_base(const float* dpool, const unsigned char* argmax, const float* base, const float* mask, int Hp,
+                                                  int Wp, int ldy, const ssd_conv_geom* g, float* wgrad_planes, float* dgrad_planes_out,
+                                                  float* bias_partial, void* stream) {
+    if (!g || !base || !mask) return SSD_ERR_NULL;
+    if (!ssd_aligned16(base) || !ssd_aligned16(mask)) return SSD_ERR_ALIGN;
+    PoolSrc ps;
+    const int e = pool_src(g, ldy, dpool, argmax, mask, Hp, Wp, &ps);
+    if (e != SSD_OK) return e;
+    if (g->H != 2 * Hp || g->W != 2 * Wp) return SSD_ERR_BAD_SHAPE;
+    ps.gate = nullptr; ps.base = base; ps.mask = mask;
+    return dy_transform(dpool, ldy, g, wgrad_planes, dgrad_planes_out, bias_partial, &ps, stream);
 }
 
 extern "C" int ssd_conv3x3_wino_wgrad_planes_pooled(const float* planes, const float* dpool, const unsigned char* argmax, const float* y_pooled,
@@ -1610,19 +1700,9 @@
     hipStream_t st = (hipStream_t)stream;
     float* Zs = static_cast<float*>(workspace);
     if (int e = launch_wgrad_tn(wgrad_planes, x_planes, Zs, g, ldy, w, st)) return e;
-    const size_t total = (size_t)g->Co * g->Ci;
-    int ks_left = w.ks;
-    if (w.ks > 1 && total / 4 < 65536) {
-        hipLaunchKernelGGL(wino_splitk_sum_kernel, dim3(grid_for(total / 4 * w.P)), dim3(256), 0, st, Zs, total, w.P, w.ks);
-        SSD_CHECK_LAUNCH();
-        ks_left = 1;
-    }
     const int blocks = dbias ? dy_bias_blocks_for(g, ldy, w.tiles) : 0;
     if (dbias && blocks == 0) return SSD_ERR_BAD_SHAPE;
-    const int nfin = grid_for(total / 4), ldp = (g->Co + 3) / 4 * 4;
-    const BiasTail bt{dbias ? bias_partial : nullptr, dbias, blocks, g->Co, ldp};
-    hipLaunchKernelGGL(wino4_wgrad_finish_kernel, dim3(nfin + (dbias ? (ldp + 15) / 16 : 0)), dim3(256), 0, st, Zs, dw_oihw, g->Co, g->Ci, ks_left,
-                       (size_t)w.ks * total, nfin, bt);
+    launch_wgrad_finish(Zs, dw_oihw, g, w.ks, BiasTail{dbias ? bias_partial : nullptr, dbias, blocks, g->Co, (g->Co + 3) / 4 * 4}, st);
     SSD_CHECK_LAUNCH();
     return SSD_OK;
 }
diff --git a/objectdetection_ssd_amd/ops.py b/objectdetection_ssd_amd/ops.py
--- a/objectdetection_ssd_amd/ops.py
+++ b/objectdetection_ssd_amd/ops.py
@@ -1344,6 +1344,8 @@
 def conv2d_wgrad_wino(x: Optional[torch.Tensor], dy: torch.Tensor, g: ConvGeom, ldy: int, want_bias: bool = True, mo: int = 2,
                       planes: Optional[torch.Tensor] = None, dgrad_planes: bool = False,
                       dw_out: Optional[torch.Tensor] = None, db_out: Optional[torch.Tensor] = None):
+    if isinstance(dy, PooledGrad) and dy.base is not None:
+        dy = dy.materialize()
     pooled = isinstance(dy, PooledGrad)
     if pooled and planes is None:
         raise ValueError("conv2d_wgrad_wino: a pooled gradient needs the kept forward planes")
@@ -1384,6 +1386,8 @@
 
 
 def wino_dy_transform(dy: torch.Tensor, g: ConvGeom, ldy: int, dgrad_planes: bool = True, want_bias: bool = True):
+    if isinstance(dy, PooledGrad) and dy.base is not None and (g.H != 2 * dy.dpool.shape[1] or g.W != 2 * dy.dpool.shape[2]):
+        dy = dy.materialize()
     pooled = isinstance(dy, PooledGrad)
     dev = dy.dpool.device if pooled else _req(dy, "dy").device
     tiles = wino_planes_shape(g)[1]
@@ -1393,7 +1397,13 @@
     Y = torch.empty((36, tiles, ldy), device=dev, dtype=torch.float32)
     Vd = torch.empty((36, tiles, ldy), device=dev, dtype=torch.float32) if dgrad_planes else None
     part = torch.empty((lib.ssd_wino4_bias_partial_floats(C.byref(g), ldy),), device=dev, dtype=torch.float32) if want_bias else None
-    if pooled:
+    if pooled and dy.base is not None:
+        if dy.in_shape != (g.N, g.H, g.W, g.Co) or ldy != g.Co:
+            raise ValueError("pooled gradient does not match the geometry")
+        check(lib.ssd_wino4_dy_transform_pooled_base(dy.dpool.data_ptr(), dy.argmax.data_ptr(), dy.base.data_ptr(), dy.mask.data_ptr(),
+                                                     dy.dpool.shape[1], dy.dpool.shape[2], ldy, C.byref(g), Y.data_ptr(), _ptr(Vd), _ptr(part),
+                                                     _stream()), "wino_dy_transform_pooled_base")
+    elif pooled:
         check(lib.ssd_wino4_dy_transform_pooled(*_pooled_args(dy, g, ldy), ldy, C.byref(g), Y.data_ptr(), _ptr(Vd), _ptr(part), _stream()),
               "wino_dy_transform_pooled")
     else:
@@ -1481,13 +1491,26 @@
 
 class PooledGrad:
 
-    def __init__(self, dpool: torch.Tensor, argmax: torch.Tensor, y_pooled: torch.Tensor, in_shape):
-        _req(dpool, "dpool"); _req(y_pooled, "y_pooled"); _req(argmax, "argmax", torch.uint8)
-        if tuple(dpool.shape) != tuple(y_pooled.shape) or tuple(argmax.shape) != tuple(dpool.shape) or dpool.shape[3] != in_shape[3]:
+    def __init__(self, dpool: torch.Tensor, argmax: torch.Tensor, y_pooled: Optional[torch.Tensor], in_shape,
+                 base: Optional[torch.Tensor] = None, mask: Optional[torch.Tensor] = None):
+        _req(dpool, "dpool"); _req(argmax, "argmax", torch.uint8)
+        if (base is None) != (mask is None) or (base is None) == (y_pooled is None):
+            raise ValueError("PooledGrad: either the pooled output (the gate) or a base gradient with the full-resolution ReLU mask")
+        if base is None:
+            _req(y_pooled, "y_pooled")
+        else:
+            _req(base, "base"); _req(mask, "mask")
+            if tuple(base.shape) != tuple(in_shape) or mask.numel() != base.numel():
+                raise ValueError("PooledGrad: base and mask must have the shape of the pool's input")
+        if (base is None and tuple(dpool.shape) != tuple(y_pooled.shape)) or tuple(argmax.shape) != tuple(dpool.shape) or dpool.shape[3] != in_shape[3]:
             raise ValueError("PooledGrad: dpool, argmax and the pooled output must have one shape, and the channels of the pool's input")
-        self.dpool, self.argmax, self.y_pooled, self.in_shape = dpool, argmax, y_pooled, tuple(in_shape)
+        self.dpool, self.argmax, self.y_pooled, self.in_shape, self.base, self.mask = dpool, argmax, y_pooled, tuple(in_shape), base, mask
 
     def materialize(self, dx: Optional[torch.Tensor] = None) -> torch.Tensor:
+        if self.base is not None:
+            if dx is not None and dx is not self.base:
+                raise ValueError("PooledGrad: a gradient with a base materialises in place in its base")
+            return maxpool_bwd(self.dpool, self.argmax, self.in_shape, 2, 2, 0, self.base, self.mask, True)
         return maxpool_bwd(self.dpool, self.argmax, self.in_shape, 2, 2, 0, dx, y_gate=self.y_pooled)
 
 
```

Result: no change. 1624, median of 6 (+0.6%).
